# uw-x/AcousticSwarms-Speech

Measured on AMD Instinct MI355X. Metric: TDoA candidates/sec (shift+normalise+spot forward+energies), higher is better.
Workload: dtype f32 via f16x3 split-operand MFMA (fp32 accumulate); 1 GPU; configs[2] scene: 5-speaker reverberant mixture (image sources), 7 mics, T=48000 samples (BASELINE's '3 s @ 16 kHz' sample count; the reference pipeline and this scene generator run at 48 kHz, where it is a 1 s clip -- the reference-native 3 s is extras.T144000), fine-stage (Strict=1) candidate batch of one mixture, FULL spot net 47.27 M params, seeded random weights; internal_batch=256, parallelism=candidate-shard x1

## Files before the change

acousticswarms-speech_amd/csrc/asw_common.h:

```cpp
#pragma once
#include <hip/hip_runtime.h>

#include <cstdarg>
#include <cstdio>
#include <cstring>

#include "../../include/asw_hip.h"

namespace asw {

char* err_buf();
int set_error(int code, const char* fmt, ...);

#define ASW_CHECK_ARG(cond, ...)                                   \
  do {                                                             \
    if (!(cond)) return ::asw::set_error(ASW_ERR_ARG, __VA_ARGS__); \
  } while (0)

#define ASW_HIP(call)                                                                 \
  do {                                                                                \
    hipError_t _e = (call);                                                           \
    if (_e != hipSuccess)                                                             \
      return ::asw::set_error(ASW_ERR_HIP, "%s failed: %s (%s:%d)", #call,            \
                              hipGetErrorString(_e), __FILE__, __LINE__);             \
  } while (0)

#define ASW_LAUNCH_CHECK()                                                            \
  do {                                                                                \
    hipError_t _e = hipGetLastError();                                                \
    if (_e != hipSuccess)                                                             \
      return ::asw::set_error(ASW_ERR_HIP, "kernel launch failed: %s (%s:%d)",        \
                              hipGetErrorString(_e), __FILE__, __LINE__);             \
  } while (0)

static inline hipStream_t as_stream(void* s) { return reinterpret_cast<hipStream_t>(s); }

struct SmemAttr {
  static constexpr int kMaxDev = 64;
  size_t bytes[kMaxDev] = {};
  int ensure(const void* kern, size_t want);
};
static inline int cdiv(long a, long b) { return (int)((a + b - 1) / b); }

#ifdef __HIPCC__
__device__ __forceinline__ float gn_glu_value(float a, float g, float m0, float r0, float m1, float r1, float ga, float ba,
                                              float gg, float bg) {
  const float av = __fmaf_rn(__fmul_rn(__fsub_rn(a, m0), r0), ga, ba);
  const float gv = __fmaf_rn(__fmul_rn(__fsub_rn(g, m1), r1), gg, bg);
  const float e = __builtin_amdgcn_exp2f(__fmul_rn(gv, -1.4426950408889634f));
  return __fmul_rn(av, __builtin_amdgcn_rcpf(__fadd_rn(1.0f, e)));
}
#endif

}

#include <string>
namespace asw {
std::string prof_name(const char* base, int bm, int bn, int bk, bool ln, bool stats);
bool prof_detail();
struct ProfScope {
  ProfScope(hipStream_t s, const std::string& name, double work, double bytes = 0.0);
  ~ProfScope();
  int slot;
  hipStream_t stream;
};
}
```

acousticswarms-speech_amd/csrc/model_common.h:

```cpp
#pragma once
#include <cstdlib>
#include <iterator>
#include <map>
#include <memory>
#include <string>
#include <vector>

#include "asw_common.h"

namespace asw_model {

struct DevBuf {
  float* p = nullptr;
  size_t n = 0;
  DevBuf() = default;
  DevBuf(const DevBuf&) = delete;
  DevBuf& operator=(const DevBuf&) = delete;
  DevBuf(DevBuf&& o) noexcept : p(o.p), n(o.n) { o.p = nullptr; o.n = 0; }
  ~DevBuf() { if (p) (void)hipFree(p); }
  int upload(const std::vector<float>& h) {
    if (p) { (void)hipFree(p); p = nullptr; }
    n = h.size();
    if (hipMalloc(&p, n * sizeof(float)) != hipSuccess) return asw::set_error(ASW_ERR_NOMEM, "hipMalloc(%zu floats)", n);
    ASW_HIP(hipMemcpy(p, h.data(), n * sizeof(float), hipMemcpyHostToDevice));
    return ASW_OK;
  }
};

struct WBuf {
  DevBuf f32;
  uint16_t* hi = nullptr;
  uint16_t* lo = nullptr;
  int32_t shift = 0;
  WBuf() = default;
  WBuf(const WBuf&) = delete;
  WBuf& operator=(const WBuf&) = delete;
  WBuf(WBuf&& o) noexcept : f32(std::move(o.f32)), hi(o.hi), lo(o.lo), shift(o.shift), fhi(o.fhi), flo(o.flo) {
    o.hi = o.lo = o.fhi = o.flo = nullptr;
  }
  ~WBuf() {
    if (hi) (void)hipFree(hi);
    if (lo) (void)hipFree(lo);
    if (fhi) (void)hipFree(fhi);
    if (flo) (void)hipFree(flo);
  }
  int upload_gemm(const std::vector<float>& h, int N, int K) {
    int rc = upload(h);
    if (rc) return rc;
    if (N % 32 == 0 && K % 16 == 0 && (size_t)N * K == h.size()) return upload_frags(h, N, K);
    return ASW_OK;
  }
  int upload(const std::vector<float>& h) {
    int rc = f32.upload(h);
    if (rc) return rc;
    std::vector<uint16_t> vh(h.size()), vl(h.size());
    if ((rc = asw_split_weights_f16(h.data(), h.size(), vh.data(), vl.data(), &shift))) return rc;
    if (hi) { (void)hipFree(hi); hi = nullptr; }
    if (lo) { (void)hipFree(lo); lo = nullptr; }
    if (hipMalloc(&hi, h.size() * 2) != hipSuccess || hipMalloc(&lo, h.size() * 2) != hipSuccess)
      return asw::set_error(ASW_ERR_NOMEM, "hipMalloc(%zu halves)", h.size());
    ASW_HIP(hipMemcpy(hi, vh.data(), h.size() * 2, hipMemcpyHostToDevice));
    ASW_HIP(hipMemcpy(lo, vl.data(), h.size() * 2, hipMemcpyHostToDevice));
    return ASW_OK;
  }
  uint16_t* fhi = nullptr;
  uint16_t* flo = nullptr;
  int upload_frags(const std::vector<float>& h, int N, int K) {
    std::vector<uint16_t> vh(h.size()), vl(h.size());
    int32_t sh = 0;
    int rc = asw_pack_fragments_f16(h.data(), N, K, vh.data(), vl.data(), &sh);
    if (rc) return rc;
    if (sh != shift) return asw::set_error(ASW_ERR_STATE, "fragment pack: inconsistent weight shift");
    if (fhi) { (void)hipFree(fhi); fhi = nullptr; }
    if (flo) { (void)hipFree(flo); flo = nullptr; }
    if (hipMalloc(&fhi, h.size() * 2) != hipSuccess || hipMalloc(&flo, h.size() * 2) != hipSuccess)
      return asw::set_error(ASW_ERR_NOMEM, "hipMalloc(%zu halves)", h.size());
    ASW_HIP(hipMemcpy(fhi, vh.data(), h.size() * 2, hipMemcpyHostToDevice));
    ASW_HIP(hipMemcpy(flo, vl.data(), h.size() * 2, hipMemcpyHostToDevice));
    return ASW_OK;
  }
  void bind(asw_convgemm_args& a, int precision) const {
    a.Wt = f32.p; a.Wt_hi = hi; a.Wt_lo = lo; a.w_shift = shift; a.precision = precision;
    a.Wf_hi = fhi; a.Wf_lo = flo;
  }
};

struct ResLayer { WBuf wt; DevBuf bias, g, b; int dil = 1; };

inline std::vector<float> pack_conv(const std::vector<float>& w, int N, int Cin, int K, const float* in_gate) {
  std::vector<float> o((size_t)N * Cin * K);
  for (int n = 0; n < N; ++n)
    for (int c = 0; c < Cin; ++c)
      for (int k = 0; k < K; ++k)
        o[((size_t)n * K + k) * Cin + c] = w[((size_t)n * Cin + c) * K + k] * (in_gate ? in_gate[c] : 1.f);
  return o;
}


inline int pack_res_layers(const std::map<std::string, std::vector<float>>& raw, const std::string& p, int ch, int K,
                           int n_layers, int dil_factor, std::vector<ResLayer>& out) {
  out.clear();
  out.resize(n_layers);
  int dil = 1;
  for (int j = 0; j < n_layers; ++j) {
    const std::string q = p + ".res.seq." + std::to_string(j);
    int rc;
    {
      const std::vector<float> packed = pack_conv(raw.at(q + ".conv.weight"), ch, ch, K, nullptr);
      if ((rc = out[j].wt.upload(packed))) return rc;
      if (ch % 32 == 0 && (ch * K) % 16 == 0 && (rc = out[j].wt.upload_frags(packed, ch, ch * K))) return rc;
    }
    if ((rc = out[j].bias.upload(raw.at(q + ".conv.bias")))) return rc;
    if ((rc = out[j].g.upload(raw.at(q + ".norm.weight")))) return rc;
    if ((rc = out[j].b.upload(raw.at(q + ".norm.bias")))) return rc;
    out[j].dil = dil;
    dil *= dil_factor;
  }
  return ASW_OK;
}

struct Arena {
  char* base;
  size_t off = 0, cap;
  bool dry;
  Arena(char* b, size_t c, bool d) : base(b), cap(c), dry(d) {}
  template <typename T>
  T* take(size_t n) {
    off = (off + 255) & ~(size_t)255;
    T* p = reinterpret_cast<T*>(base + off);
    off += n * sizeof(T);
    return p;
  }
};


struct GluSrc { const float* raw; const float* mr; const float* gamma; const float* beta; float* side_out = nullptr; };

inline bool glu_on_load_ok(const std::vector<ResLayer>& res, int prec, int ch) {
  static const int max_c = getenv("ASW_GLU_ON_LOAD_MAX_C") ? atoi(getenv("ASW_GLU_ON_LOAD_MAX_C")) : 512;
  return prec >= 1 && (ch == 64 || ch == 128 || ch == 256 || ch == 512) && ch <= max_c && !res.empty() &&
         res[0].dil == 1 && res[0].wt.fhi && res[0].wt.flo;
}

inline bool resstack_ok(const std::vector<ResLayer>& res, int prec, int ch, int K) {
  static const bool off = getenv("ASW_NO_RESSTACK") != nullptr;
  if (off || prec < 1 || ch != 64 || K % 2 == 0 || K < 3 || K > 15) return false;
  for (const ResLayer& r : res)
    if (!r.wt.fhi || !r.wt.flo) return false;
  return true;
}

inline int run_res(const std::vector<ResLayer>& res, int prec, int B, int T, int ch, int K, float* x, float* p, float* q,
            float** final_out, hipStream_t s, const GluSrc* glu = nullptr) {
  const float* in = glu ? glu->raw : x;
  float* outb = p;
  if (resstack_ok(res, prec, ch, K)) {
    static const bool nofuse = getenv("ASW_RESSTACK_NOFUSE") != nullptr;
    size_t j = 0;
    while (j < res.size()) {
      size_t n = 1;
      int halo = 0;
      while (!nofuse && j + n < res.size() && n < 3) {
        const int pad = res[j + n].dil * (K - 1) / 2;
        if (halo + pad > 64) break;
        halo += pad;
        ++n;
      }
      asw_resstack_args a = {};
      a.x = (glu && j == 0) ? nullptr : in;
      a.out = outb;
      a.B = B; a.T = T; a.C = ch; a.taps = K; a.n_layers = (int)n; a.precision = prec; a.ln_eps = 1e-5f;
      for (size_t i = 0; i < n; ++i) {
        const ResLayer& r = res[j + i];
        a.layer[i].Wf_hi = r.wt.fhi; a.layer[i].Wf_lo = r.wt.flo; a.layer[i].w_shift = r.wt.shift;
        a.layer[i].bias = r.bias.p; a.layer[i].ln_gamma = r.g.p; a.layer[i].ln_beta = r.b.p; a.layer[i].dil = r.dil;
      }
      if (glu && j == 0) {
        a.glu_raw = glu->raw; a.glu_mr = glu->mr; a.glu_gamma = glu->gamma; a.glu_beta = glu->beta; a.glu_out = glu->side_out;
      }
      int rc = asw_resstack64_f16x3(&a, s);
      if (rc) return rc;
      in = outb;
      outb = (outb == p) ? q : p;
      j += n;
    }
    *final_out = const_cast<float*>(in);
    return ASW_OK;
  }
  for (size_t j = 0; j < res.size(); ++j) {
    asw_convgemm_args a = {};
    a.A = in; res[j].wt.bind(a, prec); a.bias = res[j].bias.p; a.resid = in;
    if (glu && j == 0) {
      a.glu_raw = glu->raw; a.glu_mr = glu->mr; a.glu_gamma = glu->gamma; a.glu_beta = glu->beta; a.glu_out = glu->side_out;
    }
    a.ln_gamma = res[j].g.p; a.ln_beta = res[j].b.p; a.out = outb;
    a.B = B; a.M_out = T; a.N = ch; a.Cin = ch; a.taps = K; a.stride = 1; a.dil = res[j].dil;
    a.pad = (res[j].dil * (K - 1) + 1) / 2;
    a.a_row_stride = ch; a.a_batch_stride = (int64_t)T * ch; a.a_len = (int64_t)T * ch;
    a.relu = 1; a.ln_eps = 1e-5f;
    int rc = asw_convgemm_f32(&a, s);
    if (rc) return rc;
    in = outb;
    outb = (outb == p) ? q : p;
  }
  *final_out = const_cast<float*>(in);
  return ASW_OK;
}

inline int linear(const float* A, const WBuf& W, int prec, const float* bias, int rows, int N, int K, int relu, const float* resid,
           const float* g, const float* b, float* out, hipStream_t s) {
  asw_convgemm_args a = {};
  a.A = A; W.bind(a, prec); a.bias = bias; a.resid = resid; a.ln_gamma = g; a.ln_beta = b; a.out = out;
  a.B = 1; a.M_out = rows; a.N = N; a.Cin = K; a.taps = 1; a.stride = 1; a.dil = 1; a.pad = 0;
  a.a_row_stride = K; a.a_batch_stride = (int64_t)rows * K; a.a_len = (int64_t)rows * K;
  a.relu = relu; a.ln_eps = 1e-5f;
  if (g && N >= 1024 && N % 256 == 0 && N <= 2048) {
    a.resid = nullptr; a.ln_gamma = nullptr; a.ln_beta = nullptr;
    int rc = asw_convgemm_f32(&a, s);
    if (rc) return rc;
    return asw_add_layernorm(out, resid, g, b, rows, N, 1e-5f, out, s);
  }
  return asw_convgemm_f32(&a, s);
}

inline void pack_conv_transpose(const std::vector<float>& w, const std::vector<float>& b, int Cin, int N, int S,
                                const float* out_gate, std::vector<float>& wt, std::vector<float>& bb) {
  wt.assign((size_t)S * N * Cin, 0.f);
  bb.assign((size_t)S * N, 0.f);
  for (int r = 0; r < S; ++r)
    for (int n = 0; n < N; ++n) {
      bb[(size_t)r * N + n] = out_gate ? b[n] * out_gate[n] : b[n];
      for (int c = 0; c < Cin; ++c) {
        const float v = w[((size_t)c * N + n) * S + r];
        wt[((size_t)r * N + n) * Cin + c] = out_gate ? v * out_gate[n] : v;
      }
    }
}


#define UP(buf, vec) if ((rc = (buf).upload(vec))) return rc

struct TrunkCfg {
  int n_mics, kernel_size, depth, stride_list[8], channels, growth, encoder_channels, encoder_kernel_size,
      encoder_stride, residual_layers, residual_dilation_factor, ffw_dim;
  template <class Cfg>
  static TrunkCfg of(const Cfg& c) {
    TrunkCfg t = {c.n_mics, c.kernel_size, c.depth, {}, c.channels, c.growth, c.encoder_channels,
                  c.encoder_kernel_size, c.encoder_stride, c.residual_layers, c.residual_dilation_factor, c.ffw_dim};
    for (int i = 0; i < 8; ++i) t.stride_list[i] = c.stride_list[i];
    return t;
  }
};

inline int check_trunk_config(const TrunkCfg& c, const char* who, const char* odd) {
  ASW_CHECK_ARG(c.depth >= 1 && c.depth <= 8, "%s: depth %d", who, c.depth);
  ASW_CHECK_ARG(c.n_mics >= 1 && c.n_mics <= 32, "%s: n_mics %d", who, c.n_mics);
  ASW_CHECK_ARG(c.channels % 64 == 0, "%s: channels=%d must be a multiple of 64 for the MFMA tiles", who, c.channels);
  ASW_CHECK_ARG(c.growth >= 1 && c.residual_layers >= 1, "%s: bad config", who);
  ASW_CHECK_ARG(c.kernel_size % 2 == 1, "%s: %s", who, odd);
  ASW_CHECK_ARG(c.encoder_channels % 128 == 0, "%s: encoder_channels must be a multiple of 128", who);
  ASW_CHECK_ARG(c.encoder_stride % 4 == 0 && c.encoder_kernel_size / 2 == c.encoder_stride && c.encoder_kernel_size <= 64,
                "%s: encoder kernel/stride %d/%d unsupported (the reference's trim [9:-8] assumes 33/16)", who,
                c.encoder_kernel_size, c.encoder_stride);
  ASW_CHECK_ARG(c.ffw_dim % 128 == 0, "%s: ffw_dim must be a multiple of 128", who);
  return ASW_OK;
}

struct EncBlock { std::vector<ResLayer> res; DevBuf bias, gn_g, gn_b; };
struct DecBlock { std::vector<ResLayer> res; DevBuf gn_g, gn_b; };
struct GatedConvs { std::vector<WBuf> down_wt, up_wt; std::vector<DevBuf> up_bias; };
struct Tap { const float* p; size_t numel; };
using ParamList = std::vector<std::pair<std::string, size_t>>;

struct TrunkPlan {
  int B, T, Tp, F, RL;
  std::vector<int> Tl;
  float *mean, *stdv, *refn;
  std::vector<float*> X, Pb, Qb, raw_dn, raw_up, st_dn, st_up, mr_dn, mr_up;
  float *Y, *D, *ywave;
};

struct Trunk {
  TrunkCfg tc;
  std::map<std::string, std::vector<float>> raw;
  std::map<std::string, Tap> taps;
  bool finalized = false;
  int device = 0;
  int precision = 0;
  bool fuse_mask = true;

  std::vector<int> enc_cin, enc_cout;
  std::vector<int> dec_cin, dec_cout, dec_stride;
  int stride_product = 1;

  DevBuf pre_w, pre_b;
  std::vector<EncBlock> enc;
  std::vector<DecBlock> dec;
  WBuf byp_wt, mask_wt, dec_wt;
  WBuf byp_wt48;
  DevBuf byp_b, mask_b;
  float out_bias = 0.f;
  int byp_k = 0;

  const std::vector<float>& P(const std::string& k) const { return raw.at(k); }

  int init_shape(const TrunkCfg& c, const char* who) {
    tc = c;
    ASW_HIP(hipGetDevice(&device));
    int cin = c.channels, ch = c.channels;
    for (int i = 0; i < c.depth; ++i) {
      ASW_CHECK_ARG(c.stride_list[i] >= 1, "%s: stride", who);
      enc_cin.push_back(cin);
      enc_cout.push_back(ch);
      stride_product *= c.stride_list[i];
      cin = ch;
      ch *= c.growth;
    }
    dec_cin.assign(enc_cout.rbegin(), enc_cout.rend());
    dec_cout.assign(enc_cin.rbegin(), enc_cin.rend());
    dec_stride.assign(std::make_reverse_iterator(c.stride_list + c.depth), std::make_reverse_iterator(c.stride_list));
    return ASW_OK;
  }
  int check_level_widths(const char* who) const {
    for (int w : enc_cin) ASW_CHECK_ARG(w <= 512 && (w & (w - 1)) == 0, "%s: level width %d must be a power of two <= 512", who, w);
    return ASW_OK;
  }

  ParamList trunk_params() const {
    ParamList v;
    const size_t K = tc.kernel_size;
    v.push_back({"preproc.weight", (size_t)tc.channels * tc.n_mics});
    v.push_back({"preproc.bias", (size_t)tc.channels});
    auto res = [&](const std::string& p, size_t ch) {
      for (int j = 0; j < tc.residual_layers; ++j) {
        const std::string q = p + ".res.seq." + std::to_string(j);
        v.push_back({q + ".conv.weight", ch * ch * K});
        v.push_back({q + ".conv.bias", ch});
        v.push_back({q + ".norm.weight", ch});
        v.push_back({q + ".norm.bias", ch});
      }
    };
    for (int i = 0; i < tc.depth; ++i) {
      const std::string p = "encoder.module_list." + std::to_string(i);
      const size_t ci = enc_cin[i], co = enc_cout[i];
      res(p, ci);
      v.push_back({p + ".conv1.weight", 2 * co * ci * K});
      v.push_back({p + ".conv1.bias", 2 * co});
      v.push_back({p + ".norm1.weight", 2 * co});
      v.push_back({p + ".norm1.bias", 2 * co});
    }
    for (int i = 0; i < tc.depth; ++i) {
      const std::string p = "decoder.module_list." + std::to_string(i);
      const size_t ci = dec_cin[i], co = dec_cout[i], s = dec_stride[i];
      v.push_back({p + ".upsample.conv.weight", ci * 2 * co * s});
      v.push_back({p + ".upsample.conv.bias", 2 * co});
      v.push_back({p + ".norm1.weight", 2 * co});
      v.push_back({p + ".norm1.bias", 2 * co});
      res(p, co);
    }
    const size_t E = tc.encoder_channels, EK = tc.encoder_kernel_size;
    v.push_back({"reference_bypass.weight", E * EK});
    v.push_back({"reference_bypass.bias", E});
    v.push_back({"mask_encoder.weight", E * tc.channels * EK});
    v.push_back({"mask_encoder.bias", E});
    v.push_back({"output_decoder.weight", E * EK});
    v.push_back({"output_decoder.bias", 1});
    return v;
  }

  int finalize_trunk(const char* who, const ParamList& want) {
    {
      int dev = -1;
      ASW_HIP(hipGetDevice(&dev));
      if (dev != device)
        return asw::set_error(ASW_ERR_STATE, "%s: model was created on HIP device %d, current device is %d", who, device, dev);
    }
    for (const auto& kv : want) {
      auto it = raw.find(kv.first);
      if (it == raw.end()) return asw::set_error(ASW_ERR_STATE, "state dict is missing key %s", kv.first.c_str());
      if (it->second.size() != kv.second)
        return asw::set_error(ASW_ERR_ARG, "%s: %zu elements, expected %zu", kv.first.c_str(), it->second.size(), kv.second);
    }
    if (raw.size() != want.size())
      return asw::set_error(ASW_ERR_ARG, "state dict has %zu unexpected keys", raw.size() - want.size());
    int rc;
    const int K = tc.kernel_size, RL = tc.residual_layers, RD = tc.residual_dilation_factor;
    UP(pre_w, P("preproc.weight"));
    UP(pre_b, P("preproc.bias"));
    enc.clear(); enc.resize(tc.depth);
    dec.clear(); dec.resize(tc.depth);
    for (int i = 0; i < tc.depth; ++i) {
      const std::string p = "encoder.module_list." + std::to_string(i);
      if ((rc = pack_res_layers(raw, p, enc_cin[i], K, RL, RD, enc[i].res))) return rc;
      UP(enc[i].bias, P(p + ".conv1.bias"));
      UP(enc[i].gn_g, P(p + ".norm1.weight"));
      UP(enc[i].gn_b, P(p + ".norm1.bias"));
    }
    for (int i = 0; i < tc.depth; ++i) {
      const std::string p = "decoder.module_list." + std::to_string(i);
      if ((rc = pack_res_layers(raw, p, dec_cout[i], K, RL, RD, dec[i].res))) return rc;
      UP(dec[i].gn_g, P(p + ".norm1.weight"));
      UP(dec[i].gn_b, P(p + ".norm1.bias"));
    }
    const int E = tc.encoder_channels, EK = tc.encoder_kernel_size;
    byp_k = ((EK + 31) / 32) * 32;
    {
      const std::vector<float>& w = P("reference_bypass.weight");
      std::vector<float> wt((size_t)E * byp_k, 0.f);
      for (int n = 0; n < E; ++n)
        for (int k = 0; k < EK; ++k) wt[(size_t)n * byp_k + k] = w[(size_t)n * EK + k];
      UP(byp_wt, wt);
      UP(byp_b, P("reference_bypass.bias"));
      if (E % 32 == 0 && EK <= 48) {
        std::vector<float> w48((size_t)E * 48, 0.f);
        for (int n = 0; n < E; ++n)
          for (int k = 0; k < EK; ++k) w48[(size_t)n * 48 + k] = w[(size_t)n * EK + k];
        if ((rc = byp_wt48.upload_gemm(w48, E, 48))) return rc;
      }
    }
    if ((rc = mask_wt.upload_gemm(pack_conv(P("mask_encoder.weight"), E, tc.channels, EK, nullptr), E, tc.channels * EK))) return rc;
    UP(mask_b, P("mask_encoder.bias"));
    {
      const std::vector<float>& w = P("output_decoder.weight");
      std::vector<float> wt((size_t)64 * E, 0.f);
      for (int j = 0; j < EK; ++j)
        for (int e = 0; e < E; ++e) wt[(size_t)j * E + e] = w[(size_t)e * EK + j];
      if ((rc = dec_wt.upload_gemm(wt, 64, E))) return rc;
      out_bias = P("output_decoder.bias")[0];
    }
    return ASW_OK;
  }

  template <class Gate>
  int pack_gated(GatedConvs& o, Gate gate) const {
    const int K = tc.kernel_size;
    int rc;
    o.down_wt.clear(); o.down_wt.resize(tc.depth);
    o.up_wt.clear(); o.up_wt.resize(tc.depth);
    o.up_bias.clear(); o.up_bias.resize(tc.depth);
    for (int i = 0; i < tc.depth; ++i) {
      const std::string p = "encoder.module_list." + std::to_string(i);
      const std::vector<float> g = gate(p);
      const int n = 2 * enc_cout[i], ci = enc_cin[i];
      if ((rc = o.down_wt[i].upload_gemm(pack_conv(P(p + ".conv1.weight"), n, ci, K, g.empty() ? nullptr : g.data()), n, ci * K)))
        return rc;
    }
    for (int j = 0; j < tc.depth; ++j) {
      const std::string p = "decoder.module_list." + std::to_string(j);
      const std::vector<float> g = gate(p);
      const int ci = dec_cin[j], co2 = 2 * dec_cout[j], s = dec_stride[j];
      std::vector<float> wt, bb;
      pack_conv_transpose(P(p + ".upsample.conv.weight"), P(p + ".upsample.conv.bias"), ci, co2, s,
                          g.empty() ? nullptr : g.data(), wt, bb);
      if ((rc = o.up_wt[j].upload_gemm(wt, s * co2, ci))) return rc;
      UP(o.up_bias[j], bb);
    }
    return ASW_OK;
  }

  bool fused_mask_path() const {
    return fuse_mask && precision >= 1 && tc.encoder_channels % 256 == 0 && tc.channels % 32 == 0 &&
           tc.encoder_kernel_size <= 48 && tc.encoder_stride % 4 == 0 && byp_wt48.fhi && dec_wt.fhi && mask_wt.fhi;
  }
  void layout_levels(int B, int T, Arena& a, TrunkPlan& pl) const {
    const int depth = tc.depth, EK = tc.encoder_kernel_size, ES = tc.encoder_stride;
    pl.B = B; pl.T = T;
    pl.Tp = ((T - 1) / stride_product + 1) * stride_product;
    pl.F = (pl.Tp + 2 * (EK / 2) - EK) / ES + 1;
    pl.RL = ((EK / 2 + pl.Tp + byp_k + 64) + 3) & ~3;
    pl.Tl.assign(depth + 1, pl.Tp);
    for (int i = 0; i < depth; ++i) pl.Tl[i + 1] = pl.Tl[i] / tc.stride_list[i];
    pl.mean = a.take<float>(B);
    pl.stdv = a.take<float>(B);
    pl.refn = a.take<float>((size_t)B * pl.RL);
    pl.X.resize(depth + 1); pl.Pb.resize(depth); pl.Qb.resize(depth);
    pl.raw_dn.resize(depth); pl.raw_up.resize(depth); pl.st_dn.resize(depth); pl.st_up.resize(depth);
    pl.mr_up.resize(depth); pl.mr_dn.resize(depth);
    for (int i = 0; i <= depth; ++i) {
      const int ch = i == 0 ? tc.channels : enc_cout[i - 1];
      pl.X[i] = a.take<float>((size_t)B * pl.Tl[i] * ch);
    }
    for (int i = 0; i < depth; ++i) {
      const size_t n = (size_t)B * pl.Tl[i] * enc_cin[i];
      pl.Pb[i] = a.take<float>(n);
      pl.Qb[i] = a.take<float>(n);
      pl.raw_dn[i] = a.take<float>((size_t)B * pl.Tl[i + 1] * 2 * enc_cout[i]);
      pl.st_dn[i] = a.take<float>((size_t)B * 4 * asw_convgemm_stats_tiles(pl.Tl[i + 1], 2 * enc_cout[i]));
      pl.mr_dn[i] = a.take<float>((size_t)B * 4);
    }
    for (int j = 0; j < depth; ++j) {
      const int lvl = depth - j;
      const int s = dec_stride[j], co2 = 2 * dec_cout[j];
      pl.raw_up[j] = a.take<float>((size_t)B * pl.Tl[lvl] * s * co2);
      pl.st_up[j] = a.take<float>((size_t)B * 4 * asw_convgemm_stats_tiles(pl.Tl[lvl], s * co2));
      pl.mr_up[j] = a.take<float>((size_t)B * 4);
    }
  }
  void layout_mask(Arena& a, TrunkPlan& pl) const {
    const int E = tc.encoder_channels;
    const bool fused = fused_mask_path();
    pl.Y = fused ? nullptr : a.take<float>((size_t)pl.B * pl.F * E);
    pl.D = a.take<float>((size_t)(fused ? E / 256 : 1) * pl.B * pl.F * 64);
    pl.ywave = a.take<float>((size_t)pl.B * pl.T);
  }

  int encode(TrunkPlan& pl, const GatedConvs& g, hipStream_t s) {
    const int B = pl.B, K = tc.kernel_size;
    taps.clear();
    taps["preproc"] = {pl.X[0], (size_t)B * pl.Tl[0] * tc.channels};
    int rc;
    GluSrc src = {};
    bool glu = false;
    for (int i = 0; i < tc.depth; ++i) {
      float* r = nullptr;
      if ((rc = run_res(enc[i].res, precision, B, pl.Tl[i], enc_cin[i], K, pl.X[i], pl.Pb[i], pl.Qb[i], &r, s,
                        glu ? &src : nullptr)))
        return rc;
      asw_convgemm_args a = {};
      a.A = r; g.down_wt[i].bind(a, precision); a.bias = enc[i].bias.p; a.out = pl.raw_dn[i]; a.stats = pl.st_dn[i];
      a.B = B; a.M_out = pl.Tl[i + 1]; a.N = 2 * enc_cout[i]; a.Cin = enc_cin[i]; a.taps = K;
      a.stride = tc.stride_list[i]; a.dil = 1; a.pad = K / 2;
      a.a_row_stride = a.Cin; a.a_batch_stride = (int64_t)pl.Tl[i] * a.Cin; a.a_len = a.a_batch_stride;
      a.chan_mod = a.N;
      if ((rc = asw_convgemm_f32(&a, s))) return rc;
      glu = fuse_mask && i + 1 < tc.depth && glu_on_load_ok(enc[i + 1].res, precision, enc_cout[i]);
      const int tiles = asw_convgemm_stats_tiles(a.M_out, a.N);
      if (glu) {
        if ((rc = asw_gn_finalize(pl.st_dn[i], tiles, B, pl.Tl[i + 1], enc_cout[i], 1e-5f, pl.mr_dn[i], s))) return rc;
        src = {pl.raw_dn[i], pl.mr_dn[i], enc[i].gn_g.p, enc[i].gn_b.p, pl.X[i + 1]};
      } else if ((rc = asw_gn_glu(pl.raw_dn[i], pl.st_dn[i], tiles, enc[i].gn_g.p, enc[i].gn_b.p, B, pl.Tl[i + 1],
                                  enc_cout[i], 1e-5f, pl.X[i + 1], s))) {
        return rc;
      }
      taps["enc" + std::to_string(i)] = {pl.X[i + 1], (size_t)B * pl.Tl[i + 1] * enc_cout[i]};
    }
    return ASW_OK;
  }

  int decode(TrunkPlan& pl, const GatedConvs& g, const float*& x, hipStream_t s) {
    const int B = pl.B, K = tc.kernel_size;
    int rc;
    for (int j = 0; j < tc.depth; ++j) {
      const int lvl = tc.depth - j, ci = dec_cin[j], co = dec_cout[j], st = dec_stride[j];
      asw_convgemm_args a = {};
      a.A = x; a.A2 = pl.X[lvl]; g.up_wt[j].bind(a, precision); a.bias = g.up_bias[j].p; a.out = pl.raw_up[j];
      a.stats = pl.st_up[j];
      a.B = B; a.M_out = pl.Tl[lvl]; a.N = st * 2 * co; a.Cin = ci; a.taps = 1; a.stride = 1; a.dil = 1; a.pad = 0;
      a.a_row_stride = ci; a.a_batch_stride = (int64_t)pl.Tl[lvl] * ci; a.a_len = a.a_batch_stride;
      a.chan_mod = 2 * co;
      if ((rc = asw_convgemm_f32(&a, s))) return rc;
      const int To = pl.Tl[lvl] * st;
      const int tiles = asw_convgemm_stats_tiles(a.M_out, a.N);
      float* gb = pl.Qb[lvl - 1];
      float* r = nullptr;
      if (fuse_mask && glu_on_load_ok(dec[j].res, precision, co)) {
        if ((rc = asw_gn_finalize(pl.st_up[j], tiles, B, To, co, 1e-5f, pl.mr_up[j], s))) return rc;
        const GluSrc src = {pl.raw_up[j], pl.mr_up[j], dec[j].gn_g.p, dec[j].gn_b.p, co > 64 ? gb : nullptr};
        if ((rc = run_res(dec[j].res, precision, B, To, co, K, gb, pl.Pb[lvl - 1], gb, &r, s, &src))) return rc;
      } else {
        if ((rc = asw_gn_glu(pl.raw_up[j], pl.st_up[j], tiles, dec[j].gn_g.p, dec[j].gn_b.p, B, To, co, 1e-5f, gb, s)))
          return rc;
        if ((rc = run_res(dec[j].res, precision, B, To, co, K, gb, pl.Pb[lvl - 1], gb, &r, s))) return rc;
      }
      x = r;
      taps["dec" + std::to_string(j)] = {x, (size_t)B * To * co};
    }
    return ASW_OK;
  }

  int mask_path(TrunkPlan& pl, const float* x, const float* mean, const float* stdv, float* out_wave, hipStream_t s) {
    const int B = pl.B, C = tc.channels, E = tc.encoder_channels, EK = tc.encoder_kernel_size, ES = tc.encoder_stride;
    int rc;
    asw_convgemm_args me = {};
    me.A = x; mask_wt.bind(me, precision); me.bias = mask_b.p;
    me.B = B; me.M_out = pl.F; me.N = E; me.Cin = C; me.taps = EK; me.stride = ES; me.dil = 1; me.pad = EK / 2;
    me.a_row_stride = C; me.a_batch_stride = (int64_t)pl.Tp * C; me.a_len = me.a_batch_stride;
    if (fused_mask_path()) {
      asw_maskpath_args f = {};
      f.enc = me;
      f.ref = pl.refn; f.ref_batch_stride = pl.RL; f.ref_len = pl.RL; f.ref_hop = ES;
      f.byp_k = 48; f.byp_taps = EK; f.byp_shift = byp_wt48.shift; f.byp_hi = byp_wt48.fhi; f.byp_lo = byp_wt48.flo;
      f.byp_bias = byp_b.p;
      f.dec_hi = dec_wt.fhi; f.dec_lo = dec_wt.flo; f.dec_shift = dec_wt.shift; f.dec_taps = EK;
      f.taps = pl.D;
      if ((rc = asw_mask_path_f16x3(&f, s))) return rc;
      return asw_overlap_add_parts(pl.D, E / 256, B, pl.F, 64, EK, EK / 2, pl.T, 9, 8, out_bias, mean, stdv, out_wave, s);
    }
    {
      asw_convgemm_args a = {};
      a.A = pl.refn; byp_wt.bind(a, precision); a.bias = byp_b.p; a.out = pl.Y;
      a.B = B; a.M_out = pl.F; a.N = E; a.Cin = byp_k; a.taps = 1; a.stride = 1; a.dil = 1; a.pad = 0;
      a.a_row_stride = ES; a.a_batch_stride = pl.RL; a.a_len = pl.RL; a.relu = 1;
      if ((rc = asw_convgemm_f32(&a, s))) return rc;
    }
    me.mul = pl.Y; me.out = pl.Y; me.relu = 1;
    if ((rc = asw_convgemm_f32(&me, s))) return rc;
    taps["latent"] = {pl.Y, (size_t)B * pl.F * E};
    {
      asw_convgemm_args a = {};
      a.A = pl.Y; dec_wt.bind(a, precision); a.out = pl.D;
      a.B = B; a.M_out = pl.F; a.N = 64; a.Cin = E; a.taps = 1; a.stride = 1; a.dil = 1; a.pad = 0;
      a.a_row_stride = E; a.a_batch_stride = (int64_t)pl.F * E; a.a_len = a.a_batch_stride;
      if ((rc = asw_convgemm_f32(&a, s))) return rc;
    }
    return asw_overlap_add_unnorm(pl.D, B, pl.F, 64, EK, EK / 2, pl.T, 9, 8, out_bias, mean, stdv, out_wave, s);
  }
};

inline int check_ready(const Trunk* m, const char* fin) {
  if (!m) return asw::set_error(ASW_ERR_ARG, "null model handle");
  if (!m->finalized) return asw::set_error(ASW_ERR_STATE, "%s() has not been called", fin);
  int dev = -1;
  ASW_HIP(hipGetDevice(&dev));
  if (dev != m->device)
    return asw::set_error(ASW_ERR_STATE, "model lives on HIP device %d but the current device is %d", m->device, dev);
  return ASW_OK;
}

inline int set_precision(Trunk* m, const char* who, int precision) {
  ASW_CHECK_ARG(m && (precision >= 0 && precision <= 2), "%s: 0 (f32), 1 (f16x3) or 2 (single-pass f16)", who);
  m->precision = precision;
  return ASW_OK;
}

inline int set_param(Trunk* m, const char* who, const char* key, const float* host_data, size_t numel) {
  ASW_CHECK_ARG(m && key && host_data, "%s: null pointer", who);
  m->raw[key].assign(host_data, host_data + numel);
  m->finalized = false;
  return ASW_OK;
}

inline int get_tap(const Trunk* m, const char* who, const char* name, float* dst, size_t capacity, size_t* numel,
                   void* stream) {
  ASW_CHECK_ARG(m && name && numel, "%s: null pointer", who);
  auto it = m->taps.find(name);
  if (it == m->taps.end()) return asw::set_error(ASW_ERR_ARG, "%s: no activation named %s", who, name);
  *numel = it->second.numel;
  if (dst) {
    ASW_CHECK_ARG(capacity >= it->second.numel, "%s: buffer too small", who);
    ASW_HIP(hipMemcpyAsync(dst, it->second.p, it->second.numel * sizeof(float), hipMemcpyDeviceToDevice,
                           asw::as_stream(stream)));
  }
  return ASW_OK;
}

}
```

acousticswarms-speech_amd/csrc/prep_kernels.hip:

```cpp
#include "asw_common.h"

namespace {

constexpr int MAX_MICS = 32;

__device__ __forceinline__ float quant16(float x) {
  return rintf(x * 32768.0f) * (1.0f / 32768.0f);
}

__device__ __forceinline__ double block_sum(double v, double* red) {
#pragma unroll
  for (int o = 32; o > 0; o >>= 1) v += __shfl_xor(v, o, 64);
  const int lane = threadIdx.x & 63, wid = threadIdx.x >> 6, nw = blockDim.x >> 6;
  __syncthreads();
  if (lane == 0) red[wid] = v;
  __syncthreads();
  double s = 0.0;
  for (int i = 0; i < nw; ++i) s += red[i];
  return s;
}

__global__ __launch_bounds__(1024) void shift_stats_kernel(const float* __restrict__ mixes, int M, int T,
                                                           const int32_t* __restrict__ offsets,
                                                           const int32_t* __restrict__ mix_index, int circular,
                                                           float* __restrict__ mean_out,
                                                           float* __restrict__ std_out) {
  __shared__ int off[MAX_MICS];
  __shared__ double red[16];
  const int n = blockIdx.x;
  const float* __restrict__ mix = mixes + (mix_index ? (long)mix_index[n] * M * T : 0);
  if (threadIdx.x < M) {
    int o = threadIdx.x == 0 ? 0 : offsets[(long)n * (M - 1) + threadIdx.x - 1];
    if (circular) { o %= T; if (o < 0) o += T; }
    off[threadIdx.x] = o;
  }
  __syncthreads();
  const float inv_m = 1.0f / (float)M;
  auto ref_at = [&](int t) -> float {
    float s = 0.f;
    for (int m = 0; m < M; ++m) {
      int i = t + off[m];
      float x;
      if (circular) { if (i >= T) i -= T; x = mix[(long)m * T + i]; }
      else x = (i >= 0 && i < T) ? mix[(long)m * T + i] : 0.f;
      s += quant16(x);
    }
    return s * inv_m;
  };
  double acc = 0.0;
  for (int t = threadIdx.x; t < T; t += blockDim.x) acc += (double)ref_at(t);
  const double mean = block_sum(acc, red) / (double)T;
  acc = 0.0;
  for (int t = threadIdx.x; t < T; t += blockDim.x) {
    const double d = (double)ref_at(t) - mean;
    acc += d * d;
  }
  const double var = block_sum(acc, red) / (double)(T - 1);
  if (threadIdx.x == 0) {
    mean_out[n] = (float)mean;
    std_out[n] = (float)sqrt(var);
  }
}

template <bool SHIFTED>
__global__ __launch_bounds__(256) void preproc_kernel(const float* __restrict__ srcs, int M, int T, int T_pad,
                                                      const int32_t* __restrict__ offsets,
                                                      const int32_t* __restrict__ mix_index, int circular,
                                                      const float* __restrict__ mean, const float* __restrict__ stdv,
                                                      const float* __restrict__ w, const float* __restrict__ bias,
                                                      int C, float* __restrict__ x0, float* __restrict__ refn,
                                                      long refn_stride, int rows_per_block) {
  __shared__ int off[MAX_MICS];
  __shared__ float vs[64 * MAX_MICS];
  __shared__ float ws[128 * MAX_MICS];
  const int n = blockIdx.y;
  const float* __restrict__ src = srcs + ((SHIFTED && mix_index) ? (long)mix_index[n] * M * T : 0);
  for (int i = threadIdx.x; i < C * M; i += blockDim.x) ws[i] = w[i];
  const int c4n = C >> 2;
  if (threadIdx.x < M) {
    int o = 0;
    if (SHIFTED && threadIdx.x > 0) {
      o = offsets[(long)n * (M - 1) + threadIdx.x - 1];
      if (circular) { o %= T; if (o < 0) o += T; }
    }
    off[threadIdx.x] = o;
  }
  __syncthreads();
  const int pad = T_pad - T;
  const float mu = SHIFTED ? mean[n] : 0.f;
  const float sg = SHIFTED ? stdv[n] : 1.f;
  const int row0 = blockIdx.x * rows_per_block;
  for (int it = threadIdx.x; it < rows_per_block * M; it += blockDim.x) {
    const int m = it / rows_per_block, r = it - m * rows_per_block;
    const int tp = row0 + r;
    float x = 0.f;
    if (tp >= pad && tp < T_pad) {
      const int t = tp - pad;
      if (SHIFTED) {
        int i = t + off[m];
        if (circular) { if (i >= T) i -= T; x = src[(long)m * T + i]; }
        else x = (i >= 0 && i < T) ? src[(long)m * T + i] : 0.f;
        x = (quant16(x) - mu) / sg;
      } else {
        x = src[((long)n * M + m) * T + t];
      }
    }
    vs[r * M + m] = x;
  }
  __syncthreads();
  const int items = rows_per_block * c4n;
  for (int it = threadIdx.x; it < items; it += blockDim.x) {
    const int r = it / c4n, c4 = it - r * c4n;
    const int tp = row0 + r;
    if (tp >= T_pad) break;
    const int c = c4 * 4;
    float4 o = *reinterpret_cast<const float4*>(bias + c);
    if (tp >= pad) {
      for (int m = 0; m < M; ++m) {
        const float x = vs[r * M + m];
        o.x = fmaf(ws[(c + 0) * M + m], x, o.x);
        o.y = fmaf(ws[(c + 1) * M + m], x, o.y);
        o.z = fmaf(ws[(c + 2) * M + m], x, o.z);
        o.w = fmaf(ws[(c + 3) * M + m], x, o.w);
      }
    }
    *reinterpret_cast<float4*>(x0 + ((long)n * T_pad + tp) * C + c) = o;
    if (c4 == 0) refn[(long)n * refn_stride + tp] = vs[r * M];
  }
}

}

extern "C" int asw_shift_stats(const float* mix, int M, int T, const int32_t* offsets, int N, int circular,
                               float* mean, float* std, void* stream) {
  return asw_shift_stats_multi(mix, M, T, offsets, nullptr, N, circular, mean, std, stream);
}

extern "C" int asw_shift_stats_multi(const float* mix, int M, int T, const int32_t* offsets, const int32_t* mix_index, int N,
                                     int circular, float* mean, float* std, void* stream) {
  ASW_CHECK_ARG(mix && offsets && mean && std, "shift_stats: null pointer");
  ASW_CHECK_ARG(M >= 1 && M <= MAX_MICS && T >= 2, "shift_stats: M=%d T=%d unsupported", M, T);
  if (N == 0) return ASW_OK;
  asw::ProfScope prof(asw::as_stream(stream), "shift_stats", 0.0, (double)M * T * 4 + (double)N * 8);
  hipLaunchKernelGGL(shift_stats_kernel, dim3(N), dim3(1024), 0, asw::as_stream(stream), mix, M, T, offsets, mix_index,
                     circular, mean, std);
  ASW_LAUNCH_CHECK();
  return ASW_OK;
}

extern "C" int asw_shift_norm_preproc(const float* mix, int M, int T, int T_pad, const int32_t* offsets, int N,
                                      int circular, const float* mean, const float* std, const float* w,
                                      const float* b, int C, float* x0, float* refn, long refn_stride,
                                      void* stream) {
  return asw_shift_norm_preproc_multi(mix, M, T, T_pad, offsets, nullptr, N, circular, mean, std, w, b, C, x0, refn,
                                      refn_stride, stream);
}

extern "C" int asw_shift_norm_preproc_multi(const float* mix, int M, int T, int T_pad, const int32_t* offsets,
                                            const int32_t* mix_index, int N, int circular, const float* mean,
                                            const float* std, const float* w, const float* b, int C, float* x0, float* refn,
                                            long refn_stride, void* stream) {
  ASW_CHECK_ARG(refn_stride >= T_pad, "shift_norm_preproc: refn_stride < T_pad");
  ASW_CHECK_ARG(mix && offsets && mean && std && w && b && x0 && refn, "shift_norm_preproc: null pointer");
  ASW_CHECK_ARG(M >= 1 && M <= MAX_MICS && T >= 1 && T_pad >= T && C % 4 == 0 && C > 0 && C <= 128,
                "shift_norm_preproc: bad shape M=%d T=%d T_pad=%d C=%d (C <= 128)", M, T, T_pad, C);
  if (N == 0) return ASW_OK;
  const int rows = 64;
  dim3 grid(asw::cdiv(T_pad, rows), N);
  asw::ProfScope prof(asw::as_stream(stream), "preproc", 0.0, (double)M * T * 4 + (double)N * T_pad * (C + 1) * 4);
  hipLaunchKernelGGL(preproc_kernel<true>, grid, dim3(256), 0, asw::as_stream(stream), mix, M, T, T_pad, offsets, mix_index,
                     circular, mean, std, w, b, C, x0, refn, refn_stride, rows);
  ASW_LAUNCH_CHECK();
  return ASW_OK;
}

extern "C" int asw_pad_preproc(const float* x, int B, int M, int t, int T_pad, const float* w, const float* b,
                               int C, float* x0, float* refn, long refn_stride, void* stream) {
  ASW_CHECK_ARG(refn_stride >= T_pad, "pad_preproc: refn_stride < T_pad");
  ASW_CHECK_ARG(x && w && b && x0 && refn, "pad_preproc: null pointer");
  ASW_CHECK_ARG(M >= 1 && M <= MAX_MICS && t >= 1 && T_pad >= t && C % 4 == 0 && C > 0 && C <= 128,
                "pad_preproc: bad shape M=%d t=%d T_pad=%d C=%d (C <= 128)", M, t, T_pad, C);
  if (B == 0) return ASW_OK;
  const int rows = 64;
  dim3 grid(asw::cdiv(T_pad, rows), B);
  hipLaunchKernelGGL(preproc_kernel<false>, grid, dim3(256), 0, asw::as_stream(stream), x, M, t, T_pad,
                     (const int32_t*)nullptr, (const int32_t*)nullptr, 1, (const float*)nullptr, (const float*)nullptr, w, b, C, x0, refn,
                     refn_stride, rows);
  ASW_LAUNCH_CHECK();
  return ASW_OK;
}
```

acousticswarms-speech_amd/csrc/resstack.hip:

```cpp
#include <cstdlib>
#include <type_traits>

#include "asw_common.h"
#include "mfma_util.h"

namespace {
using namespace asw_mfma;

constexpr int RS = 272;
constexpr int C = 64;
constexpr int MAXL = 3;

struct LayerDev {
  const half8* Wh;
  const half8* Wl;
  const float* bias;
  const float* gamma;
  const float* beta;
  int dil, pad;
  int halo;
  int nfrag;
  float scale;
};

#ifdef ASW_PHASE_TIMING
__device__ unsigned long long g_rs_cycles[6] = {0, 0, 0, 0, 0, 0};
#define RS_MARK(var) const unsigned long long var = __builtin_readcyclecounter()
#else
#define RS_MARK(var)
#endif

struct KArgs {
  const float* x;
  float* out;
  const float* glu_raw;
  const float* glu_mr;
  const float* glu_gamma;
  const float* glu_beta;
  float* glu_out;
  int B, T, taps, ntile, BM, img_rows;
  float eps;
  LayerDev L[MAXL];
};

template <int NF, int QD, int NTERM>
__device__ __forceinline__ void kloop(floatx16 (&acc)[NF][2], const char* img, const int (&xb)[NF], int taps, int tapstep,
                                      const half8* __restrict__ Wh, const half8* __restrict__ Wl, int lane) {
  auto wload = [&](int kg, half8 (&h)[2], half8 (&l)[2]) {
#pragma unroll
    for (int cb = 0; cb < 2; ++cb) {
      const long o = ((long)kg * 2 + cb) * 64 + lane;
      h[cb] = Wh[o];
      if (NTERM == 3) l[cb] = Wl[o];
    }
  };
  auto xload = [&](int tap, int ks, half8 (&h)[NF], half8 (&l)[NF]) {
#pragma unroll
    for (int i = 0; i < NF; ++i) {
      const char* q = img + xb[i] + tap * tapstep + ks * 32;
      h[i] = *reinterpret_cast<const half8*>(q);
      if (NTERM == 3) l[i] = *reinterpret_cast<const half8*>(q + 128);
    }
  };
  half8 wh[QD][2], wl[QD][2];
  half8 xh[2][NF], xl[2][NF];
#pragma unroll
  for (int q = 0; q < QD; ++q) wload(q, wh[q], wl[q]);
  xload(0, 0, xh[0], xl[0]);
  const int nks = taps * 4;
  for (int tap = 0; tap < taps; ++tap) {
#pragma unroll
    for (int ks = 0; ks < 4; ++ks) {
      const int nk = (ks + 1) & 3;
      int nt = tap + (ks == 3 ? 1 : 0);
      nt = nt < taps ? nt : taps - 1;
      xload(nt, nk, xh[(ks + 1) & 1], xl[(ks + 1) & 1]);
      __builtin_amdgcn_sched_barrier(0);
      const int s = ks % QD, xbuf = ks & 1;
#pragma unroll
      for (int i = 0; i < NF; ++i)
#pragma unroll
        for (int cb = 0; cb < 2; ++cb) {
          if (NTERM == 3) {
            acc[i][cb] = __builtin_amdgcn_mfma_f32_32x32x16_f16(wh[s][cb], xl[xbuf][i], acc[i][cb], 0, 0, 0);
            acc[i][cb] = __builtin_amdgcn_mfma_f32_32x32x16_f16(wl[s][cb], xh[xbuf][i], acc[i][cb], 0, 0, 0);
          }
          acc[i][cb] = __builtin_amdgcn_mfma_f32_32x32x16_f16(wh[s][cb], xh[xbuf][i], acc[i][cb], 0, 0, 0);
        }
      int kg = tap * 4 + ks + QD;
      kg = kg < nks ? kg : nks - 1;
      wload(kg, wh[s], wl[s]);
      __builtin_amdgcn_sched_barrier(0);
    }
  }
}

template <int NL, int NW, int TM, int PH, bool POLY, bool GLU, int NTERM, int QD>
__global__ __launch_bounds__(64 * NW) __attribute__((amdgpu_waves_per_eu(TM >= 4 ? 1 : 2)))
void resstack64_kernel(const KArgs p) {
  static_assert(!POLY || NL == 1, "polyphase row sets: single layers only");
  static_assert(QD == 2 || QD == 4, "weight prefetch depth in k-steps");
  constexpr int NTHR = 64 * NW, SROWS = NTHR / 16;
  constexpr int R0 = 32 * NW * TM;
  constexpr int BMJ = R0 / PH;
  static_assert(BMJ % 32 == 0, "a row fragment must stay inside one phase");

  extern __shared__ __align__(16) char smem[];
  char* img = smem;
  float* tab = reinterpret_cast<float*>(smem + (size_t)p.img_rows * RS);

  const int tid = threadIdx.x, lane = tid & 63, wid = tid >> 6;
  const int total = p.B * p.ntile;
  const int per = (total + 7) >> 3;
  const int idx = (int)(blockIdx.x & 7) * per + (int)(blockIdx.x >> 3);
  if (idx >= total) return;
  const int b = idx / p.ntile, tile = idx - b * p.ntile;
  const int T = p.T, taps = p.taps;
  const int dil0 = p.L[0].dil, pad0 = p.L[0].pad;
  const int n_pb = POLY ? (dil0 + PH - 1) / PH : 1;
  const int jb = POLY ? tile / n_pb : 0, pb = POLY ? tile - jb * n_pb : 0;
  const int m0 = tile * p.BM;
  const int RJ = BMJ + taps - 1;
  const int R_img = POLY ? PH * RJ : R0 + 2 * pad0;

  RS_MARK(t_start);
  for (int i = tid; i < NL * 3 * 16; i += NTHR) {
    const int li = i / 48, w = (i - li * 48) / 16, c4 = i & 15;
    const float* src = w == 0 ? p.L[li].bias : w == 1 ? p.L[li].gamma : p.L[li].beta;
    reinterpret_cast<float4*>(tab)[i] = *reinterpret_cast<const float4*>(src + c4 * 4);
  }
  {
    const __amdgpu_buffer_rsrc_t rX = GLU ? act_rsrc(p.glu_raw + (long)b * T * 2 * C, (long)T * 2 * C)
                                          : act_rsrc(p.x + (long)b * T * C, (long)T * C);
    const int srow = tid >> 4, sc4 = tid & 15;
    float gm0 = 0.f, gr0 = 0.f, gm1 = 0.f, gr1 = 0.f;
    float4 gga, gba, ggg, gbg;
    if (GLU) {
      gm0 = p.glu_mr[b * 4 + 0]; gr0 = p.glu_mr[b * 4 + 1]; gm1 = p.glu_mr[b * 4 + 2]; gr1 = p.glu_mr[b * 4 + 3];
      gga = *reinterpret_cast<const float4*>(p.glu_gamma + sc4 * 4);
      gba = *reinterpret_cast<const float4*>(p.glu_beta + sc4 * 4);
      ggg = *reinterpret_cast<const float4*>(p.glu_gamma + C + sc4 * 4);
      gbg = *reinterpret_cast<const float4*>(p.glu_beta + C + sc4 * 4);
    }
    constexpr int SU = GLU ? 9 : 18;
    for (int r0 = 0; r0 < R_img; r0 += SROWS * SU) {
      float4 buf[SU];
      float4 gate[GLU ? SU : 1];
      bool okr[GLU ? SU : 1];
#pragma unroll
      for (int u = 0; u < SU; ++u) {
        const int row = r0 + u * SROWS + srow;
        int g;
        bool ok = row < R_img;
        if (!POLY) {
          g = m0 - p.L[0].halo - pad0 + row;
        } else {
          const int ph = pb * PH + row / RJ;
          const int jj = jb * BMJ + row % RJ - (taps - 1) / 2;
          g = dil0 * jj + ph;
          ok = ok && ph < dil0 && jj >= 0;
        }
        ok = ok && g >= 0 && g < T;
        if (GLU) {
          buf[u] = act_load4(rX, (long)g * 2 * C + sc4 * 4, ok);
          gate[u] = act_load4(rX, (long)g * 2 * C + C + sc4 * 4, ok);
          okr[u] = ok;
        } else {
          buf[u] = act_load4(rX, (long)g * C + sc4 * 4, ok);
        }
      }
      if (GLU) {
#pragma unroll
        for (int u = 0; u < SU; ++u) {
          float4 o;
#define ASW_GLU(f)                                                       \
  {                                                                      \
    const float gl = asw::gn_glu_value(buf[u].f, gate[u].f, gm0, gr0, gm1, gr1, gga.f, gba.f, ggg.f, gbg.f); \
    o.f = okr[u] ? gl : 0.f;                                             \
  }
          ASW_GLU(x) ASW_GLU(y) ASW_GLU(z) ASW_GLU(w)
#undef ASW_GLU
          buf[u] = o;
          if (p.glu_out && okr[u]) {
            const int g = m0 - p.L[0].halo - pad0 + r0 + u * SROWS + srow;
            if (g >= m0 && g < m0 + p.BM)
              *reinterpret_cast<float4*>(p.glu_out + ((long)b * T + g) * C + sc4 * 4) = o;
          }
        }
      }
#pragma unroll
      for (int u = 0; u < SU; ++u) {
        const int row = r0 + u * SROWS + srow;
        if (row < R_img) {
          half4 hi, lo;
          split4t<NTERM>(buf[u], hi, lo);
          *reinterpret_cast<half4*>(img + row * RS + sc4 * 8) = hi;
          *reinterpret_cast<half4*>(img + row * RS + 128 + sc4 * 8) = lo;
        }
      }
    }
  }
  __syncthreads();
  RS_MARK(t_staged);
#ifdef ASW_PHASE_TIMING
  unsigned long long t_marks[2 * MAXL + 1];
  t_marks[0] = t_staged;
#endif

  const int h = lane >> 5;
  floatx16 acc[TM][2];
  auto layer = [&](auto lic) {
    constexpr int li = decltype(lic)::value;
    constexpr bool last = li == NL - 1;
    const LayerDev& Ld = p.L[li];
    const int tapstep = (POLY ? 1 : Ld.dil) * RS;
    const int nf = Ld.nfrag - wid * TM;
#pragma unroll
    for (int i = 0; i < TM; ++i)
#pragma unroll
      for (int cb = 0; cb < 2; ++cb)
#pragma unroll
        for (int r = 0; r < 16; ++r) acc[i][cb][r] = 0.f;
    auto img_row = [&](int trow) { return POLY ? (trow / BMJ) * RJ + trow % BMJ : trow; };
    auto run = [&](auto nfc) {
      constexpr int NF = decltype(nfc)::value;
      int xb[NF];
      floatx16 a[NF][2];
#pragma unroll
      for (int i = 0; i < NF; ++i) {
        xb[i] = (img_row((wid * TM + i) * 32) + (lane & 31)) * RS + h * 16;
        a[i][0] = acc[i][0];
        a[i][1] = acc[i][1];
      }
      kloop<NF, QD, NTERM>(a, img, xb, taps, tapstep, Ld.Wh, Ld.Wl, lane);
#pragma unroll
      for (int i = 0; i < NF; ++i) { acc[i][0] = a[i][0]; acc[i][1] = a[i][1]; }
    };
    if (nf >= TM) run(std::integral_constant<int, TM>{});
    else if constexpr (TM > 1) {
      if (nf == 1) run(std::integral_constant<int, 1>{});
      if constexpr (TM > 2) {
        if (nf == 2) run(std::integral_constant<int, 2>{});
        if (nf == 3) run(std::integral_constant<int, 3>{});
      }
    }
#ifdef ASW_PHASE_TIMING
    {
      float sink = acc[0][0][0];
      asm volatile("" ::"v"(sink));
      t_marks[2 * li + 1] = __builtin_readcyclecounter();
    }
#endif
    const float* tb = tab + li * 192;
    const int cpad = POLY ? (taps - 1) / 2 : Ld.pad;
#pragma unroll
    for (int i = 0; i < TM; ++i) {
      if (i < nf) {
        const int trow = (wid * TM + i) * 32 + (lane & 31);
        const char* rrow = img + (img_row(trow) + cpad) * RS;
        float s = 0.f;
#pragma unroll
        for (int cb = 0; cb < 2; ++cb)
#pragma unroll
          for (int q = 0; q < 4; ++q) {
            const int c0 = cb * 32 + q * 8 + h * 4;
            const float4 bi = *reinterpret_cast<const float4*>(tb + c0);
            const half4 rh = *reinterpret_cast<const half4*>(rrow + c0 * 2);
            const half4 rl = *reinterpret_cast<const half4*>(rrow + 128 + c0 * 2);
            const float bv[4] = {bi.x, bi.y, bi.z, bi.w};
#pragma unroll
            for (int j = 0; j < 4; ++j) {
              float v = fmaxf(acc[i][cb][q * 4 + j] * Ld.scale + bv[j], 0.f);
              v += (float)rh[j] + (float)rl[j];
              acc[i][cb][q * 4 + j] = v;
              s += v;
            }
          }
        s += __shfl_xor(s, 32, 64);
        const float mean = s * (1.0f / C);
        float d = 0.f;
#pragma unroll
        for (int cb = 0; cb < 2; ++cb)
#pragma unroll
          for (int r = 0; r < 16; ++r) { const float cx = acc[i][cb][r] - mean; d += cx * cx; }
        d += __shfl_xor(d, 32, 64);
        const float rstd = 1.0f / sqrtf(d * (1.0f / C) + p.eps);
#pragma unroll
        for (int cb = 0; cb < 2; ++cb)
#pragma unroll
          for (int q = 0; q < 4; ++q) {
            const int c0 = cb * 32 + q * 8 + h * 4;
            const float4 g4 = *reinterpret_cast<const float4*>(tb + 64 + c0);
            const float4 b4 = *reinterpret_cast<const float4*>(tb + 128 + c0);
            const float gv[4] = {g4.x, g4.y, g4.z, g4.w}, be[4] = {b4.x, b4.y, b4.z, b4.w};
#pragma unroll
            for (int j = 0; j < 4; ++j) acc[i][cb][q * 4 + j] = (acc[i][cb][q * 4 + j] - mean) * rstd * gv[j] + be[j];
          }
      }
    }
    if constexpr (!last) {
      __syncthreads();
#pragma unroll
      for (int i = 0; i < TM; ++i) {
        if (i < nf) {
          const int trow = (wid * TM + i) * 32 + (lane & 31);
          const int t = m0 - Ld.halo + trow;
          const bool inside = t >= 0 && t < T;
          char* wrow = img + trow * RS;
#pragma unroll
          for (int cb = 0; cb < 2; ++cb)
#pragma unroll
            for (int q = 0; q < 4; ++q) {
              const int c0 = cb * 32 + q * 8 + h * 4;
              float4 v = make_float4(acc[i][cb][q * 4 + 0], acc[i][cb][q * 4 + 1], acc[i][cb][q * 4 + 2], acc[i][cb][q * 4 + 3]);
              if (!inside) v = make_float4(0.f, 0.f, 0.f, 0.f);
              half4 hi, lo;
              split4t<NTERM>(v, hi, lo);
              *reinterpret_cast<half4*>(wrow + c0 * 2) = hi;
              *reinterpret_cast<half4*>(wrow + 128 + c0 * 2) = lo;
            }
        }
      }
      __syncthreads();
    } else {
      float* __restrict__ ob = p.out + (long)b * T * C;
#pragma unroll
      for (int i = 0; i < TM; ++i) {
        if (i < nf) {
          const int trow = (wid * TM + i) * 32 + (lane & 31);
          int t;
          bool ok;
          if (!POLY) {
            t = m0 + trow;
            ok = trow < p.BM && t < T;
          } else {
            const int ph = pb * PH + trow / BMJ;
            t = dil0 * (jb * BMJ + trow % BMJ) + ph;
            ok = ph < dil0 && t < T;
          }
          if (ok) {
            float* orow = ob + (long)t * C;
#pragma unroll
            for (int cb = 0; cb < 2; ++cb)
#pragma unroll
              for (int q = 0; q < 4; ++q) {
                const int c0 = cb * 32 + q * 8 + h * 4;
                *reinterpret_cast<float4*>(orow + c0) =
                    make_float4(acc[i][cb][q * 4 + 0], acc[i][cb][q * 4 + 1], acc[i][cb][q * 4 + 2], acc[i][cb][q * 4 + 3]);
              }
          }
        }
      }
    }
  };
  layer(std::integral_constant<int, 0>{});
#ifdef ASW_PHASE_TIMING
  t_marks[2] = __builtin_readcyclecounter();
#endif
  if constexpr (NL > 1) layer(std::integral_constant<int, 1>{});
  if constexpr (NL > 2) layer(std::integral_constant<int, 2>{});
#ifdef ASW_PHASE_TIMING
  if (threadIdx.x == 0 && NL <= 2) {
    const unsigned long long t_end = __builtin_readcyclecounter();
    atomicAdd(&g_rs_cycles[0], t_staged - t_start);
    atomicAdd(&g_rs_cycles[1], t_marks[1] - t_marks[0]);
    if (NL == 1) {
      atomicAdd(&g_rs_cycles[4], t_end - t_marks[1]);
    } else {
      atomicAdd(&g_rs_cycles[2], t_marks[2] - t_marks[1]);
      atomicAdd(&g_rs_cycles[3], t_marks[3] - t_marks[2]);
      atomicAdd(&g_rs_cycles[4], t_end - t_marks[3]);
    }
    atomicAdd(&g_rs_cycles[5], 1ull);
  }
#endif
}

template <int NL, int NW, int TM, int PH, bool POLY, bool GLU, int QD>
int launch_stack(const KArgs& k, int precision, size_t smem, double flops, const char* tag, hipStream_t s) {
  const bool x1 = precision == 2;
  auto kern = x1 ? resstack64_kernel<NL, NW, TM, PH, POLY, GLU, 1, QD> : resstack64_kernel<NL, NW, TM, PH, POLY, GLU, 3, QD>;
  static asw::SmemAttr attr[2];
  if (int rc = attr[x1].ensure(reinterpret_cast<const void*>(kern), 160 * 1024)) return rc;
  const int total = k.B * k.ntile;
  dim3 grid(((total + 7) / 8) * 8);
  char nm[128];
  int nl = snprintf(nm, sizeof nm, "resstack64<%s,%dx%d%s%s>", tag, NW, TM, POLY ? (PH == 1 ? ",poly1" : PH == 2 ? ",poly2" : ",poly4") : "",
                    GLU ? ",glu" : "");
  if (asw::prof_detail()) snprintf(nm + nl, sizeof nm - nl, "[B%d M%d d%d]", k.B, k.T, k.L[0].dil);
  asw::ProfScope prof(s, nm, flops, (double)k.B * k.T * C * 4 * (GLU ? 3 : 2));
  hipLaunchKernelGGL(kern, grid, dim3(64 * NW), smem, s, k);
  ASW_LAUNCH_CHECK();
  return ASW_OK;
}

template <int NW, int TM>
int dispatch(const asw_resstack_args& a, KArgs& k, bool glu, double flops, hipStream_t s) {
  constexpr int R0 = 32 * NW * TM;
  const int dil0 = k.L[0].dil;
  const int rpp = a.T / dil0;
  if (a.n_layers == 1 && dil0 >= 7 && rpp >= 48 && !glu) {
    const int PH = rpp >= R0 - 32 ? 1 : rpp >= R0 / 2 - 32 ? 2 : 4;
    const int BMJ = R0 / PH;
    k.BM = R0;
    k.L[0].nfrag = NW * TM;
    k.ntile = asw::cdiv(asw::cdiv(a.T, dil0), BMJ) * asw::cdiv(dil0, PH);
    k.img_rows = PH * (BMJ + a.taps - 1);
    const size_t smem = (size_t)k.img_rows * RS + 3 * 64 * sizeof(float);
    switch (PH) {
      case 1: return launch_stack<1, NW, TM, 1, true, false, 4>(k, a.precision, smem, flops, "1", s);
      case 2: return launch_stack<1, NW, TM, 2, true, false, 4>(k, a.precision, smem, flops, "1", s);
      default: return launch_stack<1, NW, TM, 4, true, false, 4>(k, a.precision, smem, flops, "1", s);
    }
  }
  k.BM = R0 - 2 * k.L[0].halo;
  ASW_CHECK_ARG(k.BM >= R0 / 2, "resstack: the later layers' halo (%d rows per side) leaves %d of %d rows; fuse fewer layers",
                k.L[0].halo, k.BM, R0);
  k.ntile = asw::cdiv(a.T, k.BM);
  int rows = 0;
  for (int i = 0; i < a.n_layers; ++i) {
    k.L[i].nfrag = asw::cdiv(k.BM + 2 * k.L[i].halo, 32);
    const int r = 32 * k.L[i].nfrag + 2 * k.L[i].pad;
    rows = r > rows ? r : rows;
  }
  k.img_rows = rows;
  const size_t smem = (size_t)rows * RS + (size_t)a.n_layers * 3 * 64 * sizeof(float);
  ASW_CHECK_ARG(smem <= 160 * 1024, "resstack: image of %d rows exceeds LDS (dilation %d x %d taps too wide for a contiguous tile)",
                rows, dil0, a.taps);
  switch (a.n_layers) {
    case 1: return glu ? launch_stack<1, NW, TM, 1, false, true, 4>(k, a.precision, smem, flops, "1", s)
                       : launch_stack<1, NW, TM, 1, false, false, 4>(k, a.precision, smem, flops, "1", s);
    case 2: return glu ? launch_stack<2, NW, TM, 1, false, true, 4>(k, a.precision, smem, flops, "2", s)
                       : launch_stack<2, NW, TM, 1, false, false, 4>(k, a.precision, smem, flops, "2", s);
    default: return glu ? launch_stack<3, NW, TM, 1, false, true, 4>(k, a.precision, smem, flops, "3", s)
                        : launch_stack<3, NW, TM, 1, false, false, 4>(k, a.precision, smem, flops, "3", s);
  }
}

}

#ifdef ASW_PHASE_TIMING
extern "C" int asw_debug_resstack_cycles(unsigned long long* out6, int reset) {
  ASW_HIP(hipMemcpyFromSymbol(out6, HIP_SYMBOL(g_rs_cycles), 6 * sizeof(unsigned long long)));
  if (reset) {
    const unsigned long long z[6] = {0, 0, 0, 0, 0, 0};
    ASW_HIP(hipMemcpyToSymbol(HIP_SYMBOL(g_rs_cycles), z, sizeof z));
  }
  return ASW_OK;
}
#endif

extern "C" int asw_resstack64_f16x3(const asw_resstack_args* args, void* stream) {
  ASW_CHECK_ARG(args != nullptr, "resstack: null args");
  const asw_resstack_args& a = *args;
  hipStream_t s = asw::as_stream(stream);
  ASW_CHECK_ARG(a.C == C, "resstack: C=%d (64 only)", a.C);
  ASW_CHECK_ARG(a.n_layers >= 1 && a.n_layers <= MAXL, "resstack: 1..%d layers", MAXL);
  ASW_CHECK_ARG(a.taps >= 3 && a.taps <= 15 && a.taps % 2 == 1, "resstack: taps=%d (odd, 3..15)", a.taps);
  ASW_CHECK_ARG(a.precision == 1 || a.precision == 2, "resstack: precision 1 (f16x3) or 2 (single-pass f16)");
  ASW_CHECK_ARG(a.B > 0 && a.B <= (1 << 20) && a.T > 0 && (int64_t)a.T * 2 * C < ((int64_t)1 << 29), "resstack: bad B / T");
  ASW_CHECK_ARG(a.out && (a.x || a.glu_raw), "resstack: null tensor");
  const bool glu = a.glu_raw != nullptr;
  if (glu) ASW_CHECK_ARG(a.glu_mr && a.glu_gamma && a.glu_beta, "resstack: GroupNorm + GLU on load needs the statistics / affine arrays");
  KArgs k = {};
  k.x = a.x; k.out = a.out; k.glu_raw = a.glu_raw; k.glu_mr = a.glu_mr; k.glu_gamma = a.glu_gamma; k.glu_beta = a.glu_beta;
  k.glu_out = glu ? a.glu_out : nullptr;
  k.B = a.B; k.T = a.T; k.taps = a.taps; k.eps = a.ln_eps;
  int halo = 0;
  for (int i = a.n_layers - 1; i >= 0; --i) {
    const asw_reslayer_desc& d = a.layer[i];
    ASW_CHECK_ARG(d.Wf_hi && d.Wf_lo && d.bias && d.ln_gamma && d.ln_beta && d.dil >= 1, "resstack: layer %d incomplete", i);
    LayerDev& L = k.L[i];
    L.Wh = reinterpret_cast<const half8*>(d.Wf_hi); L.Wl = reinterpret_cast<const half8*>(d.Wf_lo);
    L.bias = d.bias; L.gamma = d.ln_gamma; L.beta = d.ln_beta;
    L.dil = d.dil; L.pad = d.dil * (a.taps - 1) / 2; L.halo = halo;
    L.scale = ldexpf(1.0f, -d.w_shift);
    halo += L.pad;
  }
  const double flops = 2.0 * a.B * (double)a.T * C * C * a.taps * a.n_layers;
  static const int tile_env = getenv("ASW_RESSTACK_TILE") ? atoi(getenv("ASW_RESSTACK_TILE")) : 0;
  const int variant = tile_env == 24 || tile_env == 44 || tile_env == 82 ? tile_env : 42;
  switch (variant) {
    case 24: return dispatch<2, 4>(a, k, glu, flops, s);
    case 44: return dispatch<4, 4>(a, k, glu, flops, s);
    case 82: return dispatch<8, 2>(a, k, glu, flops, s);
    default: return dispatch<4, 2>(a, k, glu, flops, s);
  }
}
```

acousticswarms-speech_amd/csrc/spot_model.hip:

```cpp
#include <map>
#include <memory>
#include <string>
#include <vector>

#include "model_common.h"

using namespace asw_model;

namespace {

struct TfLayer { WBuf w_in, w_out, w1, w2; DevBuf b_in, b_out, b1, b2, n1g, n1b, n2g, n2b; };
struct GateSet : GatedConvs { uint64_t stamp = 0; };

}

struct asw_spot : Trunk {
  asw_spot_config cfg;
  int batch = 32;
  uint64_t clock = 0;
  std::vector<TfLayer> tf;
  std::map<std::pair<float, float>, std::unique_ptr<GateSet>> gates;

  char* ws[2] = {nullptr, nullptr};
  size_t ws_bytes[2] = {0, 0};
  int lanes = 1;
  hipStream_t side = nullptr;
  hipEvent_t ev_fork = nullptr, ev_join = nullptr;

  ~asw_spot() {
    for (char* w : ws) if (w) (void)hipFree(w);
    if (side) (void)hipStreamDestroy(side);
    if (ev_fork) (void)hipEventDestroy(ev_fork);
    if (ev_join) (void)hipEventDestroy(ev_join);
  }
};

namespace {

ParamList expected_params(const asw_spot* m) {
  const asw_spot_config& c = m->cfg;
  ParamList v = m->trunk_params();
  for (int i = 0; i < c.depth; ++i) {
    const std::string p = "encoder.module_list." + std::to_string(i);
    v.push_back({p + ".embed1.weight", (size_t)m->enc_cin[i] * 2});
    v.push_back({p + ".embed1.bias", (size_t)m->enc_cin[i]});
  }
  for (int i = 0; i < c.depth; ++i) {
    const std::string p = "decoder.module_list." + std::to_string(i);
    v.push_back({p + ".embed1.weight", (size_t)2 * m->dec_cout[i] * 2});
    v.push_back({p + ".embed1.bias", (size_t)2 * m->dec_cout[i]});
  }
  const size_t d = m->enc_cout.back(), f = c.ffw_dim;
  for (int l = 0; l < c.num_transformer_layers; ++l) {
    const std::string p = "bottleneck.transf.layers." + std::to_string(l);
    v.push_back({p + ".self_attn.in_proj_weight", 3 * d * d});
    v.push_back({p + ".self_attn.in_proj_bias", 3 * d});
    v.push_back({p + ".self_attn.out_proj.weight", d * d});
    v.push_back({p + ".self_attn.out_proj.bias", d});
    v.push_back({p + ".linear1.weight", f * d});
    v.push_back({p + ".linear1.bias", f});
    v.push_back({p + ".linear2.weight", d * f});
    v.push_back({p + ".linear2.bias", d});
    v.push_back({p + ".norm1.weight", d});
    v.push_back({p + ".norm1.bias", d});
    v.push_back({p + ".norm2.weight", d});
    v.push_back({p + ".norm2.bias", d});
  }
  return v;
}

std::vector<float> gate_of(const std::vector<float>& w, const std::vector<float>& b, float w0, float w1) {
  std::vector<float> g(b.size());
  for (size_t c = 0; c < b.size(); ++c) g[c] = w[2 * c] * w0 + w[2 * c + 1] * w1 + b[c];
  return g;
}

int get_gates(asw_spot* m, float w0, float w1, GateSet** out) {
  auto key = std::make_pair(w0, w1);
  auto it = m->gates.find(key);
  if (it != m->gates.end()) { it->second->stamp = ++m->clock; *out = it->second.get(); return ASW_OK; }
  if (m->gates.size() >= 8) {
    auto lru = m->gates.begin();
    for (auto g = m->gates.begin(); g != m->gates.end(); ++g)
      if (g->second->stamp < lru->second->stamp) lru = g;
    m->gates.erase(lru);
  }
  std::unique_ptr<GateSet> gs(new GateSet());
  gs->stamp = ++m->clock;
  int rc = m->pack_gated(*gs, [&](const std::string& p) {
    return gate_of(m->P(p + ".embed1.weight"), m->P(p + ".embed1.bias"), w0, w1);
  });
  if (rc) return rc;
  *out = gs.get();
  m->gates[key] = std::move(gs);
  return ASW_OK;
}

struct Plan : TrunkPlan {
  float *qkv, *ctx, *x1, *ff, *ha, *hb;
  double* escr;
};

void layout(const asw_spot* m, int B, int T, Arena& a, Plan& pl) {
  m->layout_levels(B, T, a, pl);
  const size_t L = pl.Tl[m->cfg.depth], d = m->enc_cout.back(), rows = (size_t)B * L;
  pl.qkv = a.take<float>(rows * 3 * d);
  pl.ctx = a.take<float>(rows * d);
  pl.x1 = a.take<float>(rows * d);
  pl.ff = a.take<float>(rows * m->cfg.ffw_dim);
  pl.ha = a.take<float>(rows * d);
  pl.hb = a.take<float>(rows * d);
  m->layout_mask(a, pl);
  pl.escr = a.take<double>((size_t)B * (T + 1));
}

int ensure_ws(asw_spot* m, int B, int T, Plan& pl, int lane = 0) {
  Arena dry(nullptr, 0, true);
  layout(m, B, T, dry, pl);
  const size_t need = dry.off + 4096;
  if (need > m->ws_bytes[lane]) {
    size_t want = need;
    if (B < m->batch) {
      Plan full;
      Arena dry_full(nullptr, 0, true);
      layout(m, m->batch, T, dry_full, full);
      want = dry_full.off + 4096;
    }
    if (m->ws[lane]) { ASW_HIP(hipDeviceSynchronize()); (void)hipFree(m->ws[lane]); m->ws[lane] = nullptr; m->ws_bytes[lane] = 0; }
    if (hipMalloc(&m->ws[lane], want) != hipSuccess) {
      (void)hipGetLastError();
      want = need;
      if (hipMalloc(&m->ws[lane], want) != hipSuccess)
        return asw::set_error(ASW_ERR_NOMEM, "workspace of %.1f MiB for batch %d, T=%d", need / 1048576.0, B, T);
    }
    m->ws_bytes[lane] = want;
  }
  Arena real(m->ws[lane], m->ws_bytes[lane], false);
  layout(m, B, T, real, pl);
  return ASW_OK;
}

int run_network(asw_spot* m, Plan& pl, GateSet* gs, const float* mean, const float* stdv, float* out_wave,
                hipStream_t s) {
  const asw_spot_config& c = m->cfg;
  int rc;
  if ((rc = m->encode(pl, *gs, s))) return rc;
  const int L = pl.Tl[c.depth], d = m->enc_cout.back(), rows = pl.B * L;
  const float* h = pl.X[c.depth];
  for (int l = 0; l < c.num_transformer_layers; ++l) {
    TfLayer& t = m->tf[l];
    float* hout = (l % 2 == 0) ? pl.ha : pl.hb;
    if ((rc = linear(h, t.w_in, m->precision, t.b_in.p, rows, 3 * d, d, 0, nullptr, nullptr, nullptr, pl.qkv, s))) return rc;
    if ((rc = asw_attention_prec(pl.qkv, pl.B, L, d, c.num_head, m->precision, pl.ctx, s))) return rc;
    if ((rc = linear(pl.ctx, t.w_out, m->precision, t.b_out.p, rows, d, d, 0, h, t.n1g.p, t.n1b.p, pl.x1, s))) return rc;
    if ((rc = linear(pl.x1, t.w1, m->precision, t.b1.p, rows, c.ffw_dim, d, 1, nullptr, nullptr, nullptr, pl.ff, s))) return rc;
    if ((rc = linear(pl.ff, t.w2, m->precision, t.b2.p, rows, d, c.ffw_dim, 0, pl.x1, t.n2g.p, t.n2b.p, hout, s))) return rc;
    h = hout;
  }
  m->taps["bottleneck"] = {h, (size_t)rows * d};
  if ((rc = m->decode(pl, *gs, h, s))) return rc;
  return m->mask_path(pl, h, mean, stdv, out_wave, s);
}

}

extern "C" int asw_spot_create(const asw_spot_config* cfg, asw_spot** out) {
  ASW_CHECK_ARG(cfg && out, "spot_create: null pointer");
  const asw_spot_config& c = *cfg;
  const TrunkCfg tc = TrunkCfg::of(c);
  int rc = check_trunk_config(tc, "spot_create", "kernel_size must be odd");
  if (rc) return rc;
  ASW_CHECK_ARG(c.num_transformer_layers >= 0, "spot_create: bad config");
  std::unique_ptr<asw_spot> m(new asw_spot());
  m->cfg = c;
  if ((rc = m->init_shape(tc, "spot_create"))) return rc;
  const int d = m->enc_cout.back();
  ASW_CHECK_ARG(d <= 1024 && (d & (d - 1)) == 0, "spot_create: bottleneck width %d must be a power of two <= 1024", d);
  ASW_CHECK_ARG(d % c.num_head == 0 && (d / c.num_head) % 16 == 0 && d / c.num_head <= 128,
                "spot_create: head_dim %d unsupported", d / (c.num_head ? c.num_head : 1));
  if ((rc = m->check_level_widths("spot_create"))) return rc;
  *out = m.release();
  return ASW_OK;
}

extern "C" void asw_spot_destroy(asw_spot* m) { delete m; }

extern "C" int asw_spot_set_precision(asw_spot* m, int precision) { return set_precision(m, "set_precision", precision); }

extern "C" int asw_spot_set_batch(asw_spot* m, int batch) {
  ASW_CHECK_ARG(m && batch >= 1 && batch <= 4096, "set_batch: bad argument");
  m->batch = batch;
  return ASW_OK;
}

extern "C" int asw_spot_set_param(asw_spot* m, const char* key, const float* host_data, size_t numel) {
  return set_param(m, "set_param", key, host_data, numel);
}

extern "C" int asw_spot_finalize(asw_spot* m) {
  ASW_CHECK_ARG(m, "finalize: null handle");
  const asw_spot_config& c = m->cfg;
  int rc = m->finalize_trunk("finalize", expected_params(m));
  if (rc) return rc;
  m->tf.clear(); m->tf.resize(c.num_transformer_layers);
  for (int l = 0; l < c.num_transformer_layers; ++l) {
    const std::string p = "bottleneck.transf.layers." + std::to_string(l);
    TfLayer& t = m->tf[l];
    {
      const int dm = m->enc_cout.back(), ff = c.ffw_dim;
      if ((rc = t.w_in.upload_gemm(m->P(p + ".self_attn.in_proj_weight"), 3 * dm, dm))) return rc;
      if ((rc = t.w_out.upload_gemm(m->P(p + ".self_attn.out_proj.weight"), dm, dm))) return rc;
      if ((rc = t.w1.upload_gemm(m->P(p + ".linear1.weight"), ff, dm))) return rc;
      if ((rc = t.w2.upload_gemm(m->P(p + ".linear2.weight"), dm, ff))) return rc;
    }
    UP(t.b_in, m->P(p + ".self_attn.in_proj_bias"));
    UP(t.b_out, m->P(p + ".self_attn.out_proj.bias"));
    UP(t.b1, m->P(p + ".linear1.bias"));
    UP(t.b2, m->P(p + ".linear2.bias"));
    UP(t.n1g, m->P(p + ".norm1.weight")); UP(t.n1b, m->P(p + ".norm1.bias"));
    UP(t.n2g, m->P(p + ".norm2.weight")); UP(t.n2b, m->P(p + ".norm2.bias"));
  }
  m->gates.clear();
  m->finalized = true;
  return ASW_OK;
}

extern "C" int asw_spot_shift_and_sep(asw_spot* m, const float* mix, int M, int T, const int32_t* offsets, int N,
                                      int strict, int circular, float* out_wave, double* out_energy,
                                      int energy_window, void* stream) {
  return asw_spot_shift_and_sep_multi(m, mix, 1, M, T, offsets, nullptr, N, strict, circular, out_wave, out_energy,
                                      energy_window, stream);
}

extern "C" int asw_spot_shift_and_sep_multi(asw_spot* m, const float* mix, int K, int M, int T, const int32_t* offsets,
                                            const int32_t* mix_index, int N, int strict, int circular, float* out_wave,
                                            double* out_energy, int energy_window, void* stream) {
  int rc = check_ready(m, "asw_spot_finalize");
  ASW_CHECK_ARG(K >= 1 && (K == 1 || mix_index != nullptr), "shift_and_sep: K=%d mixtures need a mix_index array", K);
  if (rc) return rc;
  ASW_CHECK_ARG(N >= 0, "shift_and_sep: N=%d", N);
  if (N == 0) return ASW_OK;
  ASW_CHECK_ARG(mix && offsets, "shift_and_sep: null pointer");
  ASW_CHECK_ARG(M == m->cfg.n_mics, "shift_and_sep: mixture has %d channels, model expects %d", M, m->cfg.n_mics);
  ASW_CHECK_ARG(T >= 2, "shift_and_sep: T=%d", T);
  ASW_CHECK_ARG(out_energy == nullptr || energy_window > 0, "shift_and_sep: energy_window");
  hipStream_t s = asw::as_stream(stream);
  GateSet* gs = nullptr;
  if ((rc = get_gates(m, strict == 1 ? 1.f : 0.f, strict == 1 ? 0.f : 1.f, &gs))) return rc;
  const int Bmax = N < m->batch ? N : m->batch;
  const int n_batches = (N + Bmax - 1) / Bmax;
  const int lanes = (m->lanes == 2 && n_batches >= 2) ? 2 : 1;
  Plan pl[2];
  for (int l = 0; l < lanes; ++l)
    if ((rc = ensure_ws(m, Bmax, T, pl[l], l))) return rc;
  hipStream_t st[2] = {s, s};
  if (lanes == 2) {
    if (!m->side) {
      ASW_HIP(hipStreamCreateWithFlags(&m->side, hipStreamNonBlocking));
      ASW_HIP(hipEventCreateWithFlags(&m->ev_fork, hipEventDisableTiming));
      ASW_HIP(hipEventCreateWithFlags(&m->ev_join, hipEventDisableTiming));
    }
    st[1] = m->side;
    ASW_HIP(hipEventRecord(m->ev_fork, s));
    ASW_HIP(hipStreamWaitEvent(m->side, m->ev_fork, 0));
  }
  const int C = m->cfg.channels, pad_l = m->cfg.encoder_kernel_size / 2;
  auto batches = [&]() -> int {
    int k = 0;
    for (int i0 = 0; i0 < N; i0 += Bmax, ++k) {
      const int B = N - i0 < Bmax ? N - i0 : Bmax;
      Plan& p = pl[k % lanes];
      hipStream_t q = st[k % lanes];
      p.B = B;
      const int32_t* off = offsets + (size_t)i0 * (M - 1);
      const int32_t* mi = mix_index ? mix_index + i0 : nullptr;
      ASW_HIP(hipMemsetAsync(p.refn, 0, (size_t)B * p.RL * sizeof(float), q));
      int r;
      if ((r = asw_shift_stats_multi(mix, M, T, off, mi, B, circular, p.mean, p.stdv, q))) return r;
      if ((r = asw_shift_norm_preproc_multi(mix, M, T, p.Tp, off, mi, B, circular, p.mean, p.stdv, m->pre_w.p, m->pre_b.p, C,
                                            p.X[0], p.refn + pad_l, p.RL, q)))
        return r;
      float* y = out_wave ? out_wave + (size_t)i0 * T : p.ywave;
      if ((r = run_network(m, p, gs, p.mean, p.stdv, y, q))) return r;
      if (out_energy && (r = asw_energies(y, B, T, energy_window, p.escr, out_energy + (size_t)i0 * 2, q))) return r;
    }
    return ASW_OK;
  };
  rc = batches();
  if (lanes == 2) {
    if (hipEventRecord(m->ev_join, m->side) != hipSuccess || hipStreamWaitEvent(s, m->ev_join, 0) != hipSuccess) {
      (void)hipStreamSynchronize(m->side);
      if (!rc) rc = asw::set_error(ASW_ERR_HIP, "shift_and_sep: joining the side lane failed");
    }
  }
  return rc;
}

extern "C" int asw_spot_set_lanes(asw_spot* m, int lanes) {
  ASW_CHECK_ARG(m && (lanes == 1 || lanes == 2), "set_lanes: 1 or 2");
  m->lanes = lanes;
  return ASW_OK;
}

extern "C" int asw_spot_forward(asw_spot* m, const float* mix_norm, int B, int M, int t,
                                const float* window_embedding_host, float* out, void* stream) {
  int rc = check_ready(m, "asw_spot_finalize");
  if (rc) return rc;
  ASW_CHECK_ARG(B >= 0, "forward: B=%d", B);
  if (B == 0) return ASW_OK;
  ASW_CHECK_ARG(mix_norm && window_embedding_host && out, "forward: null pointer");
  ASW_CHECK_ARG(M == m->cfg.n_mics && t >= 1, "forward: bad shape");
  hipStream_t s = asw::as_stream(stream);
  GateSet* gs = nullptr;
  if ((rc = get_gates(m, window_embedding_host[0], window_embedding_host[1], &gs))) return rc;
  const int Bmax = B < m->batch ? B : m->batch;
  Plan pl;
  if ((rc = ensure_ws(m, Bmax, t, pl))) return rc;
  const int C = m->cfg.channels, pad_l = m->cfg.encoder_kernel_size / 2;
  for (int i0 = 0; i0 < B; i0 += Bmax) {
    const int b = B - i0 < Bmax ? B - i0 : Bmax;
    pl.B = b;
    ASW_HIP(hipMemsetAsync(pl.refn, 0, (size_t)b * pl.RL * sizeof(float), s));
    if ((rc = asw_pad_preproc(mix_norm + (size_t)i0 * M * t, b, M, t, pl.Tp, m->pre_w.p, m->pre_b.p, C, pl.X[0],
                              pl.refn + pad_l, pl.RL, s)))
      return rc;
    if ((rc = run_network(m, pl, gs, nullptr, nullptr, out + (size_t)i0 * t, s))) return rc;
  }
  return ASW_OK;
}

extern "C" int asw_spot_set_fused_mask(asw_spot* m, int on) {
  ASW_CHECK_ARG(m, "set_fused_mask: null model handle");
  m->fuse_mask = on != 0;
  return ASW_OK;
}

extern "C" int asw_spot_get_tap(asw_spot* m, const char* name, float* dst, size_t capacity, size_t* numel,
                                void* stream) {
  return get_tap(m, "get_tap", name, dst, capacity, numel, stream);
}
```

acousticswarms-speech_amd/native.py:

```python
import ctypes
import os
import subprocess
import sys
from ctypes import (POINTER, Structure, c_char_p, c_double, c_float, c_int, c_int32, c_int64,
                    c_long, c_size_t, c_void_p)

_HERE = os.path.dirname(os.path.abspath(__file__))
LIB_PATH = os.environ.get("ASW_LIB_PATH") or os.path.join(_HERE, "libasw_hip.so")
CSRC = os.path.join(_HERE, "csrc")
SOURCES = ["asw_common.cpp", "convgemm.hip", "resstack.hip", "downconv.hip", "prep_kernels.hip", "misc_kernels.hip", "attention_mfma.hip", "srp_kernels.hip",
           "pruner_kernels.hip", "geometry_kernels.hip",
           "search_host.cpp", "sep_kernels.hip", "spot_model.hip", "sep_model.hip"]
HEADERS = ["asw_common.h", "model_common.h", "mfma_util.h"]
EXTRA_FLAGS = {"geometry_kernels.hip": ["-ffp-contract=off"]}
OPS_PATH = os.path.join(_HERE, "libasw_torch_ops.so")
OPS_SOURCE = "torch_ops.cpp"


def build(force: bool = False, verbose: bool = False) -> str:
    from concurrent.futures import ThreadPoolExecutor
    hdrs = [os.path.join(CSRC, h) for h in HEADERS] + [os.path.join(os.path.dirname(_HERE), "include", "asw_hip.h")]
    hdr_time = max(os.path.getmtime(h) for h in hdrs)
    objdir = os.path.join(_HERE, "build")
    os.makedirs(objdir, exist_ok=True)
    jobs, objs = [], []
    for src in SOURCES:
        sp = os.path.join(CSRC, src)
        op = os.path.join(objdir, os.path.splitext(src)[0] + ".o")
        objs.append(op)
        if force or not os.path.exists(op) or os.path.getmtime(op) < max(os.path.getmtime(sp), hdr_time):
            jobs.append(["hipcc", "-O3", "--offload-arch=gfx950", "-std=c++17", "-fPIC"] + EXTRA_FLAGS.get(src, [])
                        + ["-c", sp, "-o", op])
    if not jobs and os.path.exists(LIB_PATH) and all(os.path.getmtime(LIB_PATH) >= os.path.getmtime(o) for o in objs):
        return LIB_PATH

    def run(cmd):
        if verbose:
            print(" ".join(cmd), file=sys.stderr)
        subprocess.run(cmd, check=True)
    with ThreadPoolExecutor(max_workers=min(6, max(1, len(jobs)))) as ex:
        list(ex.map(run, jobs))
    run(["hipcc", "--offload-arch=gfx950", "-fPIC", "-shared", "-o", LIB_PATH] + objs)
    return LIB_PATH


def build_torch_ops(force: bool = False, verbose: bool = False) -> str:
    import torch
    src = os.path.join(CSRC, OPS_SOURCE)
    hdr = os.path.join(os.path.dirname(_HERE), "include", "asw_hip.h")
    if not force and os.path.exists(OPS_PATH) and os.path.getmtime(OPS_PATH) >= max(
            os.path.getmtime(src), os.path.getmtime(hdr), os.path.getmtime(LIB_PATH)):
        return OPS_PATH
    ti = os.path.dirname(torch.__file__)
    cmd = ["hipcc", "-O2", "-std=c++17", "-fPIC", "-shared", "-D__HIP_PLATFORM_AMD__=1", "-DUSE_ROCM=1",
           f"-D_GLIBCXX_USE_CXX11_ABI={int(torch._C._GLIBCXX_USE_CXX11_ABI)}", "-w",
           f"-I{ti}/include", f"-I{ti}/include/torch/csrc/api/include", "-I/opt/rocm/include", src, "-o", OPS_PATH,
           f"-L{_HERE}", "-lasw_hip", f"-L{ti}/lib", "-ltorch", "-ltorch_cpu", "-lc10", "-lc10_hip", "-ltorch_hip",
           "-Wl,-rpath,$ORIGIN", f"-Wl,-rpath,{ti}/lib"]
    if verbose:
        print(" ".join(cmd), file=sys.stderr)
    subprocess.run(cmd, check=True)
    return OPS_PATH


class SpotConfigC(Structure):
    _fields_ = [("n_mics", c_int32), ("kernel_size", c_int32), ("depth", c_int32),
                ("stride_list", c_int32 * 8), ("channels", c_int32), ("growth", c_int32),
                ("encoder_channels", c_int32), ("encoder_kernel_size", c_int32),
                ("encoder_stride", c_int32), ("residual_layers", c_int32),
                ("residual_dilation_factor", c_int32), ("num_head", c_int32), ("ffw_dim", c_int32),
                ("num_transformer_layers", c_int32)]

    @classmethod
    def from_config(cls, cfg):
        s = cls()
        s.n_mics, s.kernel_size, s.depth = cfg.n_mics, cfg.kernel_size, cfg.depth
        for i, v in enumerate(cfg.stride_list):
            s.stride_list[i] = v
        s.channels, s.growth = cfg.channels, int(cfg.growth)
        s.encoder_channels, s.encoder_kernel_size = cfg.encoder_channels, cfg.encoder_kernel_size
        s.encoder_stride, s.residual_layers = cfg.encoder_stride, cfg.residual_layers
        s.residual_dilation_factor, s.num_head = cfg.residual_dilation_factor, cfg.num_head
        s.ffw_dim, s.num_transformer_layers = cfg.ffw_dim, cfg.num_transformer_layers
        return s


class SepConfigC(Structure):
    _fields_ = [("n_mics", c_int32), ("max_speakers", c_int32), ("kernel_size", c_int32), ("depth", c_int32),
                ("stride_list", c_int32 * 8), ("channels", c_int32), ("growth", c_int32),
                ("encoder_channels", c_int32), ("encoder_kernel_size", c_int32), ("encoder_stride", c_int32),
                ("residual_layers", c_int32), ("residual_dilation_factor", c_int32), ("num_head", c_int32),
                ("ffw_dim", c_int32), ("bottleneck_layers", c_int32), ("bottleneck_ksize", c_int32)]

    @classmethod
    def from_config(cls, cfg):
        s = cls()
        s.n_mics, s.max_speakers, s.kernel_size, s.depth = cfg.n_mics, cfg.max_speakers, cfg.kernel_size, cfg.depth
        for i, v in enumerate(cfg.stride_list):
            s.stride_list[i] = v
        s.channels, s.growth = cfg.channels, int(cfg.growth)
        s.encoder_channels, s.encoder_kernel_size = cfg.encoder_channels, cfg.encoder_kernel_size
        s.encoder_stride, s.residual_layers = cfg.encoder_stride, cfg.residual_layers
        s.residual_dilation_factor, s.num_head = cfg.residual_dilation_factor, cfg.num_head
        s.ffw_dim, s.bottleneck_layers, s.bottleneck_ksize = cfg.ffw_dim, cfg.bottleneck_layers, cfg.bottleneck_ksize
        return s


class ConvGemmArgs(Structure):
    _fields_ = [("A", c_void_p), ("A2", c_void_p), ("Wt", c_void_p), ("bias", c_void_p),
                ("resid", c_void_p), ("mul", c_void_p), ("ln_gamma", c_void_p), ("ln_beta", c_void_p),
                ("out", c_void_p), ("stats", c_void_p),
                ("B", c_int32), ("M_out", c_int32), ("N", c_int32), ("Cin", c_int32), ("taps", c_int32),
                ("stride", c_int32), ("dil", c_int32), ("pad", c_int32), ("a_row_stride", c_int32),
                ("a_batch_stride", c_int64), ("a_len", c_int64), ("chan_mod", c_int32), ("relu", c_int32),
                ("ln_eps", c_float), ("precision", c_int32), ("w_shift", c_int32), ("Wt_hi", c_void_p),
                ("Wt_lo", c_void_p), ("Wf_hi", c_void_p), ("Wf_lo", c_void_p), ("stats_stride", c_int32),
                ("glu_raw", c_void_p), ("glu_mr", c_void_p), ("glu_gamma", c_void_p), ("glu_beta", c_void_p),
                ("glu_out", c_void_p)]


class MaskPathArgs(Structure):
    _fields_ = [("enc", ConvGemmArgs), ("ref", c_void_p), ("ref_batch_stride", c_int64), ("ref_len", c_int64),
                ("ref_hop", c_int32), ("byp_k", c_int32), ("byp_taps", c_int32), ("byp_shift", c_int32),
                ("byp_hi", c_void_p), ("byp_lo", c_void_p), ("byp_bias", c_void_p), ("dec_hi", c_void_p),
                ("dec_lo", c_void_p), ("dec_shift", c_int32), ("dec_taps", c_int32), ("taps", c_void_p)]


class ResLayerDesc(Structure):
    _fields_ = [("Wf_hi", c_void_p), ("Wf_lo", c_void_p), ("bias", c_void_p), ("ln_gamma", c_void_p),
                ("ln_beta", c_void_p), ("dil", c_int32), ("w_shift", c_int32)]


class ResStackArgs(Structure):
    _fields_ = [("x", c_void_p), ("out", c_void_p), ("B", c_int32), ("T", c_int32), ("C", c_int32), ("taps", c_int32),
                ("n_layers", c_int32), ("precision", c_int32), ("ln_eps", c_float), ("layer", ResLayerDesc * 3),
                ("glu_raw", c_void_p), ("glu_mr", c_void_p), ("glu_gamma", c_void_p), ("glu_beta", c_void_p),
                ("glu_out", c_void_p)]


SIGNATURES = {
    "asw_last_error": (c_char_p, []),
    "asw_abi_version": (c_int, []),
    "asw_profile_enable": (c_int, [c_int]),
    "asw_profile_report": (c_int, [c_char_p, c_size_t]),
    "asw_spot_create": (c_int, [POINTER(SpotConfigC), POINTER(c_void_p)]),
    "asw_spot_destroy": (None, [c_void_p]),
    "asw_spot_set_param": (c_int, [c_void_p, c_char_p, c_void_p, c_size_t]),
    "asw_spot_finalize": (c_int, [c_void_p]),
    "asw_spot_set_batch": (c_int, [c_void_p, c_int]),
    "asw_spot_set_precision": (c_int, [c_void_p, c_int]),
    "asw_spot_set_lanes": (c_int, [c_void_p, c_int]),
    "asw_split_weights_f16": (c_int, [c_void_p, c_size_t, c_void_p, c_void_p, POINTER(c_int32)]),
    "asw_pack_fragments_f16": (c_int, [c_void_p, c_int, c_int, c_void_p, c_void_p, POINTER(c_int32)]),
    "asw_spot_shift_and_sep": (c_int, [c_void_p, c_void_p, c_int, c_int, c_void_p, c_int, c_int, c_int,
                                       c_void_p, c_void_p, c_int, c_void_p]),
    "asw_spot_shift_and_sep_multi": (c_int, [c_void_p, c_void_p, c_int, c_int, c_int, c_void_p, c_void_p, c_int, c_int, c_int,
                                             c_void_p, c_void_p, c_int, c_void_p]),
    "asw_spot_forward": (c_int, [c_void_p, c_void_p, c_int, c_int, c_int, POINTER(c_float), c_void_p, c_void_p]),
    "asw_spot_set_fused_mask": (c_int, [c_void_p, c_int]),
    "asw_spot_get_tap": (c_int, [c_void_p, c_char_p, c_void_p, c_size_t, POINTER(c_size_t), c_void_p]),
    "asw_sep_create": (c_int, [POINTER(SepConfigC), POINTER(c_void_p)]),
    "asw_sep_destroy": (None, [c_void_p]),
    "asw_sep_set_param": (c_int, [c_void_p, c_char_p, c_void_p, c_size_t]),
    "asw_sep_finalize": (c_int, [c_void_p]),
    "asw_sep_set_precision": (c_int, [c_void_p, c_int]),
    "asw_sep_infer": (c_int, [c_void_p, c_void_p, c_int, c_int, c_void_p, c_int, c_void_p, c_void_p]),
    "asw_sep_forward": (c_int, [c_void_p, c_void_p, c_int, c_int, c_int, c_int, c_void_p, c_void_p]),
    "asw_sep_forward_counts": (c_int, [c_void_p, c_void_p, c_int, c_int, c_int, c_int, c_void_p, c_void_p, c_void_p]),
    "asw_sep_get_config": (c_int, [c_void_p, POINTER(SepConfigC)]),
    "asw_sep_get_tap": (c_int, [c_void_p, c_char_p, c_void_p, c_size_t, POINTER(c_size_t), c_void_p]),
    "asw_joint_shift_stats": (c_int, [c_void_p, c_int, c_int, c_void_p, c_int, c_void_p, c_void_p, c_void_p, c_void_p]),
    "asw_joint_shift_stats_scratch_doubles": (c_int, []),
    "asw_add_layernorm2": (c_int, [c_void_p, c_void_p, c_float, c_void_p, c_void_p, c_int, c_int, c_float, c_int,
                                   c_void_p, c_void_p, c_void_p]),
    "asw_glu_rows": (c_int, [c_void_p, c_long, c_int, c_void_p, c_void_p]),
    "asw_dwconv_ln_swish": (c_int, [c_void_p, c_void_p, c_void_p, c_void_p, c_void_p, c_int, c_int, c_int, c_int,
                                    c_float, c_void_p, c_void_p]),
    "asw_relpos_attention": (c_int, [c_void_p, c_void_p, c_void_p, c_void_p, c_int, c_int, c_int, c_int, c_float,
                                     c_void_p, c_void_p]),
    "asw_inter_attention": (c_int, [c_void_p, c_int, c_int, c_int, c_int, c_int, c_void_p, c_void_p]),
    "asw_shift_stats": (c_int, [c_void_p, c_int, c_int, c_void_p, c_int, c_int, c_void_p, c_void_p, c_void_p]),
    "asw_shift_norm_preproc": (c_int, [c_void_p, c_int, c_int, c_int, c_void_p, c_int, c_int, c_void_p, c_void_p,
                                       c_void_p, c_void_p, c_int, c_void_p, c_void_p, c_long, c_void_p]),
    "asw_shift_stats_multi": (c_int, [c_void_p, c_int, c_int, c_void_p, c_void_p, c_int, c_int, c_void_p, c_void_p, c_void_p]),
    "asw_shift_norm_preproc_multi": (c_int, [c_void_p, c_int, c_int, c_int, c_void_p, c_void_p, c_int, c_int, c_void_p,
                                             c_void_p, c_void_p, c_void_p, c_int, c_void_p, c_void_p, c_long, c_void_p]),
    "asw_pad_preproc": (c_int, [c_void_p, c_int, c_int, c_int, c_int, c_void_p, c_void_p, c_int, c_void_p,
                                c_void_p, c_long, c_void_p]),
    "asw_convgemm_f32": (c_int, [POINTER(ConvGemmArgs), c_void_p]),
    "asw_mask_path_f16x3": (c_int, [POINTER(MaskPathArgs), c_void_p]),
    "asw_resstack64_f16x3": (c_int, [POINTER(ResStackArgs), c_void_p]),
    "asw_convgemm_stats_tiles": (c_int, [c_int, c_int]),
    "asw_f16x3_overflow_count": (c_int, [c_int, POINTER(c_int32)]),
    "asw_gn_glu": (c_int, [c_void_p, c_void_p, c_int, c_void_p, c_void_p, c_int, c_int, c_int, c_float, c_void_p,
                           c_void_p]),
    "asw_gn_finalize": (c_int, [c_void_p, c_int, c_int, c_int, c_int, c_float, c_void_p, c_void_p]),
    "asw_attention": (c_int, [c_void_p, c_int, c_int, c_int, c_int, c_void_p, c_void_p]),
    "asw_attention_prec": (c_int, [c_void_p, c_int, c_int, c_int, c_int, c_int, c_void_p, c_void_p]),
    "asw_overlap_add_unnorm": (c_int, [c_void_p, c_int, c_int, c_int, c_int, c_int, c_int, c_int, c_int, c_float,
                                       c_void_p, c_void_p, c_void_p, c_void_p]),
    "asw_overlap_add_parts": (c_int, [c_void_p, c_int, c_int, c_int, c_int, c_int, c_int, c_int, c_int, c_int, c_float,
                                      c_void_p, c_void_p, c_void_p, c_void_p]),
    "asw_energies": (c_int, [c_void_p, c_int, c_int, c_int, c_void_p, c_void_p, c_void_p]),
    "asw_pair_sisdr": (c_int, [c_void_p, c_int, c_int, c_void_p, c_void_p]),
    "asw_center_rows": (c_int, [c_void_p, c_int, c_int, c_void_p]),
    "asw_segment_sisdr": (c_int, [c_void_p, c_int, c_int, c_void_p, c_void_p, c_int, c_void_p, c_void_p]),
    "asw_add_layernorm": (c_int, [c_void_p, c_void_p, c_void_p, c_void_p, c_int, c_int, c_float, c_void_p, c_void_p]),
    "asw_search_area": (c_int, [c_void_p, c_int, c_void_p, c_int, c_void_p, c_void_p, c_void_p, c_double, c_double,
                                POINTER(c_int), POINTER(c_void_p), POINTER(c_void_p), POINTER(c_void_p),
                                POINTER(c_void_p)]),
    "asw_free": (None, [c_void_p]),
    "asw_cube_select": (c_int, [c_void_p, c_int, c_int, c_int, c_int, c_int, c_int, c_int, c_int, c_void_p, c_void_p,
                                c_void_p, c_int64, POINTER(c_int64)]),
    "asw_cube_select_planes": (c_int, [c_void_p, c_int, c_int, c_int, c_int, c_int, c_int, c_int, c_int, c_void_p, c_void_p,
                                c_void_p, c_int64, POINTER(c_int64)]),
    "asw_srp_frames": (c_int, [c_int, c_int, c_int]),
    "asw_srp_cross_spectra": (c_int, [c_void_p, c_int, c_int, c_int, c_int, c_int, c_int, c_int, c_int, c_int,
                                      c_float, c_void_p, c_void_p, c_void_p, c_int, c_void_p, c_void_p, c_void_p]),
    "asw_srp_map": (c_int, [c_void_p, c_int, c_int, c_int, c_void_p, c_int, c_int, c_void_p, c_void_p, c_void_p,
                            c_void_p, c_void_p, c_void_p]),
    "asw_pruner_covariance": (c_int, [c_void_p, c_int, c_int, c_int, c_int, c_int, c_int, c_int, c_int, c_int,
                                      c_void_p, c_void_p, c_void_p]),
    "asw_hermitian_eigh": (c_int, [c_void_p, c_int, c_int, c_void_p, c_void_p, c_void_p]),
    "asw_music_map": (c_int, [c_void_p, c_int, c_int, c_int, c_void_p, c_int, c_void_p, c_void_p, c_void_p, c_void_p,
                              c_void_p]),
    "asw_tops_map": (c_int, [c_void_p, c_void_p, c_int, c_int, c_int, c_int, c_void_p, c_int, c_double, c_void_p,
                             c_void_p, c_void_p, c_void_p]),
    "asw_geom_lookup_planes": (c_int, [c_void_p, c_int, c_void_p, c_int, c_void_p, c_int, c_void_p, c_int, c_double, c_double,
                                       c_void_p, c_void_p]),
    "asw_geom_voxel_map": (c_int, [c_void_p, c_int, c_void_p, c_int, c_void_p, c_int, c_void_p, c_int, c_void_p, c_void_p,
                                   c_double, c_double, c_double, c_void_p, c_void_p, c_void_p, c_void_p]),
    "asw_geom_label": (c_int, [c_void_p, c_void_p, c_int, c_int, c_int, c_int, c_void_p, c_void_p, c_void_p, POINTER(c_int),
                               c_void_p]),
    "asw_geom_workspace_bytes": (c_int64, [c_int]),
    "asw_geom_compact": (c_int, [c_void_p, c_void_p, c_void_p, c_int, c_void_p, c_int, c_void_p, c_int, c_void_p, c_int,
                                 c_void_p, c_double, c_void_p, c_int64, c_void_p, c_void_p, c_void_p, c_void_p, c_void_p,
                                 c_void_p, c_void_p, c_void_p, c_void_p, POINTER(c_int), c_void_p]),
}

_lib = None


def lib():
    global _lib
    if _lib is None:
        if not os.path.exists(LIB_PATH):
            raise RuntimeError(
                f"{LIB_PATH} is missing: run `python -c 'import __graft_entry__ as g; g.build()'` "
                "(hipcc --offload-arch=gfx950).  There is no CPU fallback for the hot path.")
        import torch
        L = ctypes.CDLL(LIB_PATH)
        for name, (res, args) in SIGNATURES.items():
            fn = getattr(L, name)
            fn.restype = res
            fn.argtypes = args
        _lib = L
    return _lib


_ops = None


def torch_ops():
    global _ops
    if _ops is None:
        lib()
        if not os.path.exists(OPS_PATH):
            raise RuntimeError(f"{OPS_PATH} is missing: run `python -c 'import __graft_entry__ as g; g.build()'`.  "
                               "The hot path is exposed only through these custom ops; there is no fallback.")
        import torch
        torch.ops.load_library(OPS_PATH)
        _ops = torch.ops.asw
    return _ops


def check(status: int):
    if status != 0:
        msg = lib().asw_last_error()
        raise RuntimeError(f"libasw_hip: status {status}: {msg.decode() if msg else ''}")


def ptr(t):
    return None if t is None else c_void_p(t.data_ptr())


def current_stream():
    import torch
    return c_void_p(torch.cuda.current_stream().cuda_stream)


def to_device(a, device):
    import torch
    src = torch.from_numpy(a)
    host = torch.empty(src.shape, dtype=src.dtype, pin_memory=True)
    host.copy_(src)
    return host.to(device, non_blocking=True)


def to_host(t):
    import torch
    if not t.is_cuda:
        return t.numpy()
    host = torch.empty(t.shape, dtype=t.dtype, pin_memory=True)
    host.copy_(t)
    return host.numpy()
```

acousticswarms-speech_amd/ops.py:

```python
from ctypes import byref

import torch

from .native import ConvGemmArgs, MaskPathArgs, ResStackArgs, check, current_stream, lib, ptr


def _f32(t):
    assert t.is_cuda and t.dtype == torch.float32 and t.is_contiguous(), "need contiguous float32 CUDA tensor"
    return t


def pack_conv_weight(w: torch.Tensor) -> torch.Tensor:
    N, Cin, K = w.shape
    return w.permute(0, 2, 1).reshape(N, K * Cin).contiguous()


def convgemm(A, Wt, M_out, N, Cin, taps=1, stride=1, dil=1, pad=0, bias=None, relu=False, resid=None, mul=None,
             ln=None, stats_chan_mod=0, A2=None, B=None, a_row_stride=None, a_batch_stride=None, a_len=None,
             out=None, ln_eps=1e-5, precision="f32", use_fragments=True, glu=None, glu_out=None):
    _f32(A); _f32(Wt)
    if B is None:
        B = A.shape[0]
    a_row_stride = Cin if a_row_stride is None else a_row_stride
    if a_batch_stride is None:
        a_batch_stride = A[0].numel()
    if a_len is None:
        a_len = a_batch_stride
    if out is None:
        out = torch.empty((B, M_out, N), dtype=torch.float32, device=A.device)
    stats = None
    if stats_chan_mod:
        tiles = lib().asw_convgemm_stats_tiles(M_out, N)
        stats = torch.zeros((B, tiles, 4), dtype=torch.float32, device=A.device)
    a = ConvGemmArgs()
    a.A, a.A2, a.Wt = A.data_ptr(), (A2.data_ptr() if A2 is not None else None), Wt.data_ptr()
    a.bias = bias.data_ptr() if bias is not None else None
    a.resid = resid.data_ptr() if resid is not None else None
    a.mul = mul.data_ptr() if mul is not None else None
    a.ln_gamma = ln[0].data_ptr() if ln is not None else None
    a.ln_beta = ln[1].data_ptr() if ln is not None else None
    a.out = out.data_ptr()
    a.stats = stats.data_ptr() if stats is not None else None
    a.B, a.M_out, a.N, a.Cin, a.taps, a.stride, a.dil, a.pad = B, M_out, N, Cin, taps, stride, dil, pad
    a.a_row_stride, a.a_batch_stride, a.a_len = a_row_stride, a_batch_stride, a_len
    a.chan_mod, a.relu, a.ln_eps = stats_chan_mod, int(relu), ln_eps
    if glu is not None:
        a.glu_raw, a.glu_mr, a.glu_gamma, a.glu_beta = (_f32(t).data_ptr() for t in glu)
        if glu_out is not None:
            a.glu_out = _f32(glu_out).data_ptr()
    keep = None
    if precision in ("f16x3", "f16"):
        hi, lo, shift = split_weights_f16(Wt)
        keep = (hi, lo)
        a.precision, a.w_shift, a.Wt_hi, a.Wt_lo = (1 if precision == "f16x3" else 2), shift, hi.data_ptr(), lo.data_ptr()
        if use_fragments and N % 32 == 0 and (taps * Cin) % 16 == 0:
            fh, fl, sh2 = pack_fragments_f16(Wt, N, taps * Cin)
            assert sh2 == shift
            keep = keep + (fh, fl)
            a.Wf_hi, a.Wf_lo = fh.data_ptr(), fl.data_ptr()
    check(lib().asw_convgemm_f32(byref(a), current_stream()))
    torch.cuda.current_stream().synchronize() if keep is not None else None
    return out, stats


def resstack(x, layers, taps=7, precision="f16x3", eps=1e-5, glu=None, out=None, glu_out=None):
    src = x if glu is None else glu[0]
    B, T = src.shape[0], src.shape[1]
    if out is None:
        out = torch.empty((B, T, 64), dtype=torch.float32, device=src.device)
    a = ResStackArgs()
    a.x = _f32(x).data_ptr() if x is not None else None
    a.out = out.data_ptr()
    a.B, a.T, a.C, a.taps, a.n_layers = B, T, 64, taps, len(layers)
    a.precision, a.ln_eps = (1 if precision == "f16x3" else 2), eps
    keep = []
    for i, (Wt, bias, gamma, beta, dil) in enumerate(layers):
        fh, fl, sh = pack_fragments_f16(_f32(Wt), 64, taps * 64)
        keep.append((fh, fl))
        d = a.layer[i]
        d.Wf_hi, d.Wf_lo, d.w_shift, d.dil = fh.data_ptr(), fl.data_ptr(), sh, dil
        d.bias, d.ln_gamma, d.ln_beta = _f32(bias).data_ptr(), _f32(gamma).data_ptr(), _f32(beta).data_ptr()
    if glu is not None:
        a.glu_raw, a.glu_mr, a.glu_gamma, a.glu_beta = (_f32(t).data_ptr() for t in glu)
        if glu_out is not None:
            a.glu_out = _f32(glu_out).data_ptr()
    check(lib().asw_resstack64_f16x3(byref(a), current_stream()))
    torch.cuda.current_stream().synchronize()
    return out


def pack_fragments_f16(Wt, N, K):
    import ctypes
    import numpy as np
    w = np.ascontiguousarray(Wt.detach().cpu().numpy(), dtype=np.float32).reshape(N, K)
    hi = np.empty(w.size, dtype=np.uint16)
    lo = np.empty(w.size, dtype=np.uint16)
    sh = ctypes.c_int32()
    check(lib().asw_pack_fragments_f16(ctypes.c_void_p(w.ctypes.data), N, K, ctypes.c_void_p(hi.ctypes.data),
                                       ctypes.c_void_p(lo.ctypes.data), byref(sh)))
    dev = Wt.device
    return (torch.from_numpy(hi.view(np.int16)).to(dev), torch.from_numpy(lo.view(np.int16)).to(dev), sh.value)


def split_weights_f16(Wt):
    import ctypes
    import numpy as np
    w = np.ascontiguousarray(Wt.detach().cpu().numpy(), dtype=np.float32)
    hi = np.empty(w.size, dtype=np.uint16)
    lo = np.empty(w.size, dtype=np.uint16)
    sh = ctypes.c_int32()
    check(lib().asw_split_weights_f16(ctypes.c_void_p(w.ctypes.data), w.size, ctypes.c_void_p(hi.ctypes.data),
                                      ctypes.c_void_p(lo.ctypes.data), byref(sh)))
    dev = Wt.device
    return (torch.from_numpy(hi.view(np.int16)).to(dev), torch.from_numpy(lo.view(np.int16)).to(dev), sh.value)


def gn_glu(raw, stats, gamma, beta, eps=1e-5):
    B, T, C2 = raw.shape
    C = C2 // 2
    out = torch.empty((B, T, C), dtype=torch.float32, device=raw.device)
    check(lib().asw_gn_glu(ptr(_f32(raw)), ptr(_f32(stats)), stats.shape[1], ptr(_f32(gamma)), ptr(_f32(beta)),
                           B, T, C, eps, ptr(out), current_stream()))
    return out


def gn_finalize(stats, T, C, eps=1e-5):
    B = stats.shape[0]
    mr = torch.empty((B, 4), dtype=torch.float32, device=stats.device)
    check(lib().asw_gn_finalize(ptr(_f32(stats)), stats.shape[1], B, T, C, eps, ptr(mr), current_stream()))
    return mr


def add_layernorm(x, resid, gamma, beta, eps=1e-5):
    rows, N = x.shape
    out = torch.empty_like(x)
    check(lib().asw_add_layernorm(ptr(_f32(x)), ptr(_f32(resid)), ptr(_f32(gamma)), ptr(_f32(beta)), rows, N, eps,
                                  ptr(out), current_stream()))
    return out


def attention(qkv, nhead, precision="f32"):
    B, L, d3 = qkv.shape
    d = d3 // 3
    ctx = torch.empty((B, L, d), dtype=torch.float32, device=qkv.device)
    check(lib().asw_attention_prec(ptr(_f32(qkv)), B, L, d, nhead, {"f32": 0, "f16x3": 1, "f16": 2}[precision], ptr(ctx),
                                   current_stream()))
    return ctx


def shift_stats(mix, offsets, circular=True):
    M, T = mix.shape
    N = offsets.shape[0]
    mean = torch.empty((N,), dtype=torch.float32, device=mix.device)
    std = torch.empty((N,), dtype=torch.float32, device=mix.device)
    check(lib().asw_shift_stats(ptr(_f32(mix)), M, T, ptr(offsets), N, int(circular), ptr(mean), ptr(std),
                                current_stream()))
    return mean, std


def shift_norm_preproc(mix, offsets, mean, std, w, b, T_pad, circular=True):
    M, T = mix.shape
    N = offsets.shape[0]
    C = w.shape[0]
    x0 = torch.empty((N, T_pad, C), dtype=torch.float32, device=mix.device)
    refn = torch.zeros((N, T_pad), dtype=torch.float32, device=mix.device)
    check(lib().asw_shift_norm_preproc(ptr(_f32(mix)), M, T, T_pad, ptr(offsets), N, int(circular), ptr(mean),
                                       ptr(std), ptr(_f32(w)), ptr(_f32(b)), C, ptr(x0), ptr(refn), T_pad,
                                       current_stream()))
    return x0, refn


def overlap_add_unnorm(D, taps, hop, t, trim_left, trim_right, bias, mean=None, std=None):
    B, F, ldd = D.shape
    out = torch.empty((B, t), dtype=torch.float32, device=D.device)
    check(lib().asw_overlap_add_unnorm(ptr(_f32(D)), B, F, ldd, taps, hop, t, trim_left, trim_right, float(bias),
                                       ptr(mean), ptr(std), ptr(out), current_stream()))
    return out


def overlap_add_parts(Dp, taps, hop, t, trim_left, trim_right, bias, mean=None, std=None):
    nparts, B, F, ldd = Dp.shape
    out = torch.empty((B, t), dtype=torch.float32, device=Dp.device)
    check(lib().asw_overlap_add_parts(ptr(_f32(Dp)), nparts, B, F, ldd, taps, hop, t, trim_left, trim_right,
                                      float(bias), ptr(mean), ptr(std), ptr(out), current_stream()))
    return out


def mask_path(x, ref, ref_hop, enc_w, enc_b, byp_w, byp_b, dec_w, frames, stride, pad):
    B, Tp, C = x.shape
    E, _, EK = enc_w.shape
    dev = x.device
    Wt = pack_conv_weight(enc_w).to(dev)
    fh, fl, sh = pack_fragments_f16(Wt, E, EK * C)
    wb = torch.zeros((E, 48), dtype=torch.float32)
    wb[:, :byp_w.shape[-1]] = byp_w[:, 0].cpu()
    bh, bl, bsh = pack_fragments_f16(wb.to(dev), E, 48)
    wd = torch.zeros((64, E), dtype=torch.float32)
    wd[:dec_w.shape[-1]] = dec_w[:, 0].t().cpu()
    dh, dl, dsh = pack_fragments_f16(wd.to(dev), 64, E)
    parts = torch.zeros((E // 256, B, frames, 64), dtype=torch.float32, device=dev)
    m = MaskPathArgs()
    a = m.enc
    a.A, a.bias = _f32(x).data_ptr(), (_f32(enc_b).data_ptr() if enc_b is not None else None)
    a.B, a.M_out, a.N, a.Cin, a.taps, a.stride, a.dil, a.pad = B, frames, E, C, EK, stride, 1, pad
    a.a_row_stride, a.a_batch_stride, a.a_len = C, Tp * C, Tp * C
    a.precision, a.w_shift, a.Wf_hi, a.Wf_lo = 1, sh, fh.data_ptr(), fl.data_ptr()
    m.ref, m.ref_batch_stride, m.ref_len, m.ref_hop = _f32(ref).data_ptr(), ref.shape[1], ref.shape[1], ref_hop
    m.byp_k, m.byp_taps, m.byp_shift = 48, byp_w.shape[-1], bsh
    m.byp_hi, m.byp_lo = bh.data_ptr(), bl.data_ptr()
    m.byp_bias = _f32(byp_b).data_ptr() if byp_b is not None else None
    m.dec_hi, m.dec_lo, m.dec_shift, m.dec_taps = dh.data_ptr(), dl.data_ptr(), dsh, dec_w.shape[-1]
    m.taps = parts.data_ptr()
    check(lib().asw_mask_path_f16x3(byref(m), current_stream()))
    torch.cuda.current_stream().synchronize()
    return parts


def energies(y, window=12000):
    B, T = y.shape
    scratch = torch.empty((B, T + 1), dtype=torch.float64, device=y.device)
    out = torch.empty((B, 2), dtype=torch.float64, device=y.device)
    check(lib().asw_energies(ptr(_f32(y)), B, T, window, ptr(scratch), ptr(out), current_stream()))
    return out


def pair_sisdr(y):
    n, T = y.shape
    out = torch.empty((n, n), dtype=torch.float64, device=y.device)
    check(lib().asw_pair_sisdr(ptr(_f32(y)), n, T, ptr(out), current_stream()))
    return out


def joint_shift_stats(mix, offsets):
    M, T = mix.shape
    S = offsets.shape[0]
    scratch = torch.empty((lib().asw_joint_shift_stats_scratch_doubles(),), dtype=torch.float64, device=mix.device)
    mean = torch.empty((S,), dtype=torch.float32, device=mix.device)
    std = torch.empty((S,), dtype=torch.float32, device=mix.device)
    check(lib().asw_joint_shift_stats(ptr(_f32(mix)), M, T, ptr(offsets), S, ptr(scratch), ptr(mean), ptr(std),
                                      current_stream()))
    return mean, std


def add_layernorm2(x, y=None, alpha=1.0, gamma=None, beta=None, eps=1e-5, act=0, want_sum=False, want_ln=True):
    rows, N = x.shape
    s = torch.empty_like(x) if want_sum else None
    o = torch.empty_like(x) if want_ln else None
    check(lib().asw_add_layernorm2(ptr(_f32(x)), ptr(y), float(alpha), ptr(gamma), ptr(beta), rows, N, eps, act, ptr(s),
                                   ptr(o), current_stream()))
    return s, o


def glu_rows(raw):
    rows, C2 = raw.shape
    out = torch.empty((rows, C2 // 2), dtype=torch.float32, device=raw.device)
    check(lib().asw_glu_rows(ptr(_f32(raw)), rows, C2 // 2, ptr(out), current_stream()))
    return out


def dwconv_ln_swish(u, w, bias, gamma, beta, eps=1e-5):
    BS, L, d = u.shape
    K = w.shape[-1]
    wT = w.reshape(d, K).t().contiguous()
    out = torch.empty_like(u)
    check(lib().asw_dwconv_ln_swish(ptr(_f32(u)), ptr(_f32(wT)), ptr(_f32(bias)), ptr(_f32(gamma)), ptr(_f32(beta)),
                                    BS, L, d, K, eps, ptr(out), current_stream()))
    return out


def relpos_attention(qkv, P, bias_u, bias_v, nhead, scale):
    BS, L, d3 = qkv.shape
    d = d3 // 3
    ctx = torch.empty((BS, L, d), dtype=torch.float32, device=qkv.device)
    check(lib().asw_relpos_attention(ptr(_f32(qkv)), ptr(_f32(P)), ptr(_f32(bias_u)), ptr(_f32(bias_v)), BS, L, d, nhead,
                                     float(scale), ptr(ctx), current_stream()))
    return ctx


def inter_attention(qkv, nhead):
    NB, S, L, d3 = qkv.shape
    d = d3 // 3
    ctx = torch.empty((NB, S, L, d), dtype=torch.float32, device=qkv.device)
    check(lib().asw_inter_attention(ptr(_f32(qkv)), NB, S, L, d, nhead, ptr(ctx), current_stream()))
    return ctx


def f16x3_overflow_count(reset=True) -> int:
    import ctypes
    c = ctypes.c_int32()
    check(lib().asw_f16x3_overflow_count(int(reset), byref(c)))
    return int(c.value) & 0xFFFFFFFF
```

include/asw_hip.h:

```cpp
#ifndef ASW_HIP_H
#define ASW_HIP_H

#include <stddef.h>
#include <stdint.h>

#ifdef __cplusplus
extern "C" {
#endif

typedef enum asw_status {
  ASW_OK = 0,
  ASW_ERR_ARG = -1,
  ASW_ERR_HIP = -2,
  ASW_ERR_NOMEM = -3,
  ASW_ERR_STATE = -4
} asw_status;

const char* asw_last_error(void);
int asw_abi_version(void);

int asw_profile_enable(int on);
int asw_profile_report(char* buf, size_t cap);

typedef struct asw_spot_config {
  int32_t n_mics;
  int32_t kernel_size;
  int32_t depth;
  int32_t stride_list[8];
  int32_t channels;
  int32_t growth;
  int32_t encoder_channels;
  int32_t encoder_kernel_size;
  int32_t encoder_stride;
  int32_t residual_layers;
  int32_t residual_dilation_factor;
  int32_t num_head;
  int32_t ffw_dim;
  int32_t num_transformer_layers;
} asw_spot_config;

typedef struct asw_spot asw_spot;

int asw_spot_create(const asw_spot_config* cfg, asw_spot** out);
void asw_spot_destroy(asw_spot* m);

int asw_spot_set_param(asw_spot* m, const char* key, const float* host_data, size_t numel);
int asw_spot_finalize(asw_spot* m);

int asw_spot_set_batch(asw_spot* m, int batch);

int asw_spot_set_lanes(asw_spot* m, int lanes);

int asw_spot_set_precision(asw_spot* m, int precision);

int asw_spot_shift_and_sep(asw_spot* m, const float* mix, int M, int T,
                           const int32_t* offsets, int N, int strict, int circular,
                           float* out_wave, double* out_energy, int energy_window,
                           void* stream);

int asw_spot_shift_and_sep_multi(asw_spot* m, const float* mix, int K, int M, int T, const int32_t* offsets,
                                 const int32_t* mix_index, int N, int strict, int circular, float* out_wave,
                                 double* out_energy, int energy_window, void* stream);

int asw_spot_forward(asw_spot* m, const float* mix_norm, int B, int M, int t,
                     const float* window_embedding_host, float* out, void* stream);

int asw_spot_set_fused_mask(asw_spot* m, int on);

int asw_spot_get_tap(asw_spot* m, const char* name, float* dst, size_t capacity, size_t* numel,
                     void* stream);

typedef struct asw_sep_config {
  int32_t n_mics;
  int32_t max_speakers;
  int32_t kernel_size;
  int32_t depth;
  int32_t stride_list[8];
  int32_t channels;
  int32_t growth;
  int32_t encoder_channels;
  int32_t encoder_kernel_size;
  int32_t encoder_stride;
  int32_t residual_layers;
  int32_t residual_dilation_factor;
  int32_t num_head;
  int32_t ffw_dim;
  int32_t bottleneck_layers;
  int32_t bottleneck_ksize;
} asw_sep_config;

typedef struct asw_sep asw_sep;

int asw_sep_create(const asw_sep_config* cfg, asw_sep** out);
void asw_sep_destroy(asw_sep* m);
int asw_sep_set_param(asw_sep* m, const char* key, const float* host_data, size_t numel);
int asw_sep_finalize(asw_sep* m);
int asw_sep_set_precision(asw_sep* m, int precision);

int asw_sep_infer(asw_sep* m, const float* mix, int M, int T, const int32_t* offsets, int S, float* out,
                  void* stream);

int asw_sep_forward(asw_sep* m, const float* mix_norm, int B, int S, int M, int t, float* out, void* stream);
int asw_sep_forward_counts(asw_sep* m, const float* mix_norm, int B, int S, int M, int t, const int32_t* counts,
                           float* out, void* stream);
int asw_sep_get_config(const asw_sep* m, asw_sep_config* out);

int asw_sep_get_tap(asw_sep* m, const char* name, float* dst, size_t capacity, size_t* numel, void* stream);

int asw_joint_shift_stats(const float* mix, int M, int T, const int32_t* offsets, int S, double* scratch,
                          float* mean, float* std, void* stream);
int asw_joint_shift_stats_scratch_doubles(void);

int asw_add_layernorm2(const float* x, const float* y, float alpha, const float* gamma, const float* beta,
                       int rows, int N, float eps, int act, float* sum_out, float* ln_out, void* stream);

int asw_glu_rows(const float* raw, long rows, int C, float* out, void* stream);

int asw_dwconv_ln_swish(const float* u, const float* wT, const float* bias, const float* gamma, const float* beta,
                        int BS, int L, int d, int K, float eps, float* out, void* stream);

int asw_relpos_attention(const float* qkv, const float* P, const float* bias_u, const float* bias_v, int BS, int L,
                         int d, int nhead, float scale, float* ctx, void* stream);

int asw_inter_attention(const float* qkv, int NB, int S, int L, int d, int nhead, float* ctx, void* stream);


int asw_shift_stats(const float* mix, int M, int T, const int32_t* offsets, int N,
                    int circular, float* mean, float* std, void* stream);

int asw_shift_norm_preproc(const float* mix, int M, int T, int T_pad, const int32_t* offsets,
                           int N, int circular, const float* mean, const float* std,
                           const float* w, const float* b, int C, float* x0, float* refn,
                           long refn_stride, void* stream);

int asw_shift_stats_multi(const float* mix, int M, int T, const int32_t* offsets, const int32_t* mix_index, int N,
                          int circular, float* mean, float* std, void* stream);
int asw_shift_norm_preproc_multi(const float* mix, int M, int T, int T_pad, const int32_t* offsets,
                                 const int32_t* mix_index, int N, int circular, const float* mean, const float* std,
                                 const float* w, const float* b, int C, float* x0, float* refn, long refn_stride,
                                 void* stream);

int asw_pad_preproc(const float* x, int B, int M, int t, int T_pad, const float* w,
                    const float* b, int C, float* x0, float* refn, long refn_stride,
                    void* stream);

typedef struct asw_convgemm_args {
  const float* A;
  const float* A2;
  const float* Wt;
  const float* bias;
  const float* resid;
  const float* mul;
  const float* ln_gamma;
  const float* ln_beta;
  float* out;
  float* stats;
  int32_t B, M_out, N, Cin, taps, stride, dil, pad;
  int32_t a_row_stride;
  int64_t a_batch_stride;
  int64_t a_len;
  int32_t chan_mod;
  int32_t relu;
  float ln_eps;
  int32_t precision;
  int32_t w_shift;
  const void* Wt_hi;
  const void* Wt_lo;
  const void* Wf_hi;
  const void* Wf_lo;
  int32_t stats_stride;
  const float* glu_raw;
  const float* glu_mr;
  const float* glu_gamma;
  const float* glu_beta;
  float* glu_out;
} asw_convgemm_args;
int asw_pack_fragments_f16(const float* Wt, int N, int K, uint16_t* hi, uint16_t* lo, int32_t* w_shift);
int asw_convgemm_f32(const asw_convgemm_args* args, void* stream);
typedef struct asw_maskpath_args {
  asw_convgemm_args enc;
  const float* ref;
  int64_t ref_batch_stride;
  int64_t ref_len;
  int32_t ref_hop;
  int32_t byp_k;
  int32_t byp_taps;
  int32_t byp_shift;
  const void* byp_hi;
  const void* byp_lo;
  const float* byp_bias;
  const void* dec_hi;
  const void* dec_lo;
  int32_t dec_shift;
  int32_t dec_taps;
  float* taps;
} asw_maskpath_args;
int asw_mask_path_f16x3(const asw_maskpath_args* args, void* stream);
typedef struct asw_reslayer_desc {
  const void* Wf_hi;
  const void* Wf_lo;
  const float* bias;
  const float* ln_gamma;
  const float* ln_beta;
  int32_t dil;
  int32_t w_shift;
} asw_reslayer_desc;
typedef struct asw_resstack_args {
  const float* x;
  float* out;
  int32_t B, T, C, taps, n_layers;
  int32_t precision;
  float ln_eps;
  asw_reslayer_desc layer[3];
  const float* glu_raw;
  const float* glu_mr;
  const float* glu_gamma;
  const float* glu_beta;
  float* glu_out;
} asw_resstack_args;
int asw_resstack64_f16x3(const asw_resstack_args* args, void* stream);
int asw_split_weights_f16(const float* w, size_t n, uint16_t* hi, uint16_t* lo, int32_t* w_shift);
int asw_f16x3_overflow_count(int reset, uint32_t* count);
int asw_convgemm_stats_tiles(int M_out, int N);

int asw_gn_glu(const float* raw, const float* stats, int n_partials, const float* gamma,
               const float* beta, int B, int T, int C, float eps, float* out, void* stream);
int asw_gn_finalize(const float* stats, int n_partials, int B, int T, int C, float eps, float* mr, void* stream);

int asw_attention(const float* qkv, int B, int L, int d, int nhead, float* ctx, void* stream);
int asw_attention_prec(const float* qkv, int B, int L, int d, int nhead, int precision, float* ctx, void* stream);

int asw_overlap_add_unnorm(const float* D, int B, int F, int ldd, int taps, int hop,
                           int t, int trim_left, int trim_right, float bias, const float* mean,
                           const float* std, float* out, void* stream);
int asw_overlap_add_parts(const float* D, int nparts, int B, int F, int ldd, int taps, int hop,
                          int t, int trim_left, int trim_right, float bias, const float* mean,
                          const float* std, float* out, void* stream);

int asw_energies(const float* y, int B, int T, int window, double* scratch, double* out,
                 void* stream);

int asw_add_layernorm(const float* x, const float* resid, const float* gamma, const float* beta,
                      int rows, int N, float eps, float* out, void* stream);

int asw_center_rows(float* y, int B, int T, void* stream);

int asw_pair_sisdr(const float* y, int n, int T, double* out, void* stream);

int asw_segment_sisdr(const float* y, int n, int T, const int32_t* segments, const int32_t* seg_count,
                      int kmax, double* out, void* stream);

int asw_search_area(const double* points, int n_pts, const double* mic, int M, double* offset,
                    double* width, const double* ub, double sound_speed, double fs, int* n_children,
                    double** child_offset, double** child_width, int** child_count, int** child_index);
void asw_free(void* p);

int asw_cube_select(const double* offsets, int ny, int nx, int nz, int P, int y0, int y1, int x0, int x1,
                    const double* lo, const double* hi, int32_t* out_idx, int64_t cap, int64_t* count);
int asw_cube_select_planes(const double* planes, int ny, int nx, int nz, int P, int y0, int y1, int x0, int x1,
                    const double* lo, const double* hi, int32_t* out_idx, int64_t cap, int64_t* count);

int asw_srp_frames(int window, int nfft, int hop);
int asw_srp_cross_spectra(const float* mix, int M, int T, int window, int step, int n_windows,
                          int nfft, int hop, int nbins, int nb_pad, float tol,
                          const float* twiddle, const int32_t* pair_i, const int32_t* pair_j,
                          int P, float* xf_scratch, float* cc, void* stream);
int asw_srp_map(const float* cc, int n_windows, int nbins, int P, const double* tau, int G, int M,
                const double* omega, const int32_t* pair_i, const int32_t* pair_j,
                float* part_scratch, float* out, void* stream);

int asw_pruner_covariance(const float* mix, int M, int T, int window, int step, int n_windows,
                          int nfft, int hop, int bin0, int nbins, double* cov, double* magsum,
                          void* stream);
int asw_hermitian_eigh(const double* a, int n, int M, double* evals, double* evecs, void* stream);
int asw_music_map(const double* evecs, int n_windows, int nbins, int M, const double* tau, int G,
                  const double* omega, double* p_scratch, double* max_scratch, float* out,
                  void* stream);
int asw_tops_map(const double* evecs, const double* magsum, int n_windows, int nbins, int bin0,
                 int M, const double* delta, int G, double coef, double* q_scratch,
                 int32_t* max_bin, float* out, void* stream);

int asw_geom_lookup_planes(const double* ys, int ny, const double* xs, int nx, const double* zs, int nz,
                           const double* mics, int M, double C, double FS, double* planes, void* stream);
int asw_geom_voxel_map(const double* xs, int Lx, const double* ys, int Ly, const double* zs, int Lz,
                       const double* mics, int M, const double* border, const double* centre, double C,
                       double FS, double resolution, int32_t* q, uint8_t* valid, double* dis_matrix,
                       void* stream);
int asw_geom_label(const int32_t* q, const uint8_t* valid, int Lx, int Ly, int Lz, int P,
                   uint32_t* adj_scratch, int32_t* flag_scratch, int32_t* labels, int* sweeps, void* stream);
int64_t asw_geom_workspace_bytes(int n_voxels);
int asw_geom_compact(const int32_t* labels, const int32_t* q, const double* xs, int Lx, const double* ys, int Ly,
                     const double* zs, int Lz, const double* mics, int M, const double* centre, double C,
                     void* workspace, int64_t workspace_bytes, int32_t* power_index, int32_t* valid_flat,
                     int32_t* valid_cid, int32_t* members, int32_t* bounds, int32_t* offsets, double* centres,
                     double* tau, double* delta, int* counts, void* stream);

#ifdef __cplusplus
}
#endif
#endif
```

Baseline: 2383 candidates/s.

## Fuse shift/normalise preprocessing into the first encoder residual stack load

The shift, quantise, normalise and 1x1 preprocessing conv is now computed inside the first fused resstack kernel's tile-loading stage, reading the raw mixture directly. The separate preproc kernel and its full B x T x 64 activation write and read-back are skipped, and refn is written as a side output. This removes one kernel launch and a large round trip through memory at the cost of recomputing the preprocessing for halo rows and extra registers in the load stage. It is enabled by default when M<=8 and channels are 64.

Result: no change. 2397 candidates/s, median of 6 (+0.6%).

```diff
diff --git a/acousticswarms-speech_amd/csrc/asw_common.h b/acousticswarms-speech_amd/csrc/asw_common.h
--- a/acousticswarms-speech_amd/csrc/asw_common.h
+++ b/acousticswarms-speech_amd/csrc/asw_common.h
@@ -50,6 +50,20 @@
   const float e = __builtin_amdgcn_exp2f(__fmul_rn(gv, -1.4426950408889634f));
   return __fmul_rn(av, __builtin_amdgcn_rcpf(__fadd_rn(1.0f, e)));
 }
+
+__device__ __forceinline__ float quant16(float x) { return rintf(x * 32768.0f) * (1.0f / 32768.0f); }
+__device__ __forceinline__ int shifted_index(int t, int off, int T, int circular) {
+  const int i = t + off;
+  if (circular) return i >= T ? i - T : i;
+  return (i >= 0 && i < T) ? i : -1;
+}
+__device__ __forceinline__ float quant_norm(float x, float mu, float sg) { return (quant16(x) - mu) / sg; }
+__device__ __forceinline__ void preproc_fma(float4& o, float w0, float w1, float w2, float w3, float x) {
+  o.x = fmaf(w0, x, o.x);
+  o.y = fmaf(w1, x, o.y);
+  o.z = fmaf(w2, x, o.z);
+  o.w = fmaf(w3, x, o.w);
+}
 #endif
 
 }
diff --git a/acousticswarms-speech_amd/csrc/model_common.h b/acousticswarms-speech_amd/csrc/model_common.h
--- a/acousticswarms-speech_amd/csrc/model_common.h
+++ b/acousticswarms-speech_amd/csrc/model_common.h
@@ -150,8 +150,22 @@
   return true;
 }
 
+inline bool stage_fusion(char part) {
+  static const char* env = getenv("ASW_STAGE_FUSION");
+  if (!env || !*env) return true;
+  if (env[0] == '0') return false;
+  if (env[0] == 'a' || env[0] == 'A' || env[0] == 'b' || env[0] == 'B') return (env[0] | 0x20) == part;
+  return true;
+}
+
+struct PreSrc {
+  const float* mix; const int32_t* offsets; const int32_t* mix_index; const float *mean, *stdv, *w, *b;
+  float* refn; long refn_stride; int M, T, circular;
+};
+
 inline int run_res(const std::vector<ResLayer>& res, int prec, int B, int T, int ch, int K, float* x, float* p, float* q,
-            float** final_out, hipStream_t s, const GluSrc* glu = nullptr) {
+            float** final_out, hipStream_t s, const GluSrc* glu = nullptr, const PreSrc* pre = nullptr) {
+  if (pre && !resstack_ok(res, prec, ch, K)) return asw::set_error(ASW_ERR_STATE, "run_res: the preproc source needs the fused stack");
   const float* in = glu ? glu->raw : x;
   float* outb = p;
   if (resstack_ok(res, prec, ch, K)) {
@@ -166,8 +180,9 @@
         halo += pad;
         ++n;
       }
-      asw_resstack_args a = {};
-      a.x = (glu && j == 0) ? nullptr : in;
+      asw_resstack_src_args sa = {};
+      asw_resstack_args& a = sa.stack;
+      a.x = ((glu || pre) && j == 0) ? nullptr : in;
       a.out = outb;
       a.B = B; a.T = T; a.C = ch; a.taps = K; a.n_layers = (int)n; a.precision = prec; a.ln_eps = 1e-5f;
       for (size_t i = 0; i < n; ++i) {
@@ -178,7 +193,16 @@
       if (glu && j == 0) {
         a.glu_raw = glu->raw; a.glu_mr = glu->mr; a.glu_gamma = glu->gamma; a.glu_beta = glu->beta; a.glu_out = glu->side_out;
       }
-      int rc = asw_resstack64_f16x3(&a, s);
+      int rc;
+      if (pre && j == 0) {
+        sa.pre_mix = pre->mix; sa.pre_offsets = pre->offsets; sa.pre_mix_index = pre->mix_index;
+        sa.pre_mean = pre->mean; sa.pre_std = pre->stdv; sa.pre_w = pre->w; sa.pre_b = pre->b;
+        sa.pre_refn = pre->refn; sa.pre_refn_stride = pre->refn_stride;
+        sa.pre_M = pre->M; sa.pre_T = pre->T; sa.pre_circular = pre->circular;
+        rc = asw_resstack64_src_f16x3(&sa, s);
+      } else {
+        rc = asw_resstack64_f16x3(&a, s);
+      }
       if (rc) return rc;
       in = outb;
       outb = (outb == p) ? q : p;
@@ -278,6 +302,7 @@
   float *mean, *stdv, *refn;
   std::vector<float*> X, Pb, Qb, raw_dn, raw_up, st_dn, st_up, mr_dn, mr_up;
   float *Y, *D, *ywave;
+  const PreSrc* pre = nullptr;
 };
 
 struct Trunk {
@@ -504,17 +529,21 @@
     pl.ywave = a.take<float>((size_t)pl.B * pl.T);
   }
 
+  bool preproc_on_load_ok(int M) const {
+    return stage_fusion('a') && M <= 8 && tc.channels == 64 && resstack_ok(enc[0].res, precision, tc.channels, tc.kernel_size);
+  }
+
   int encode(TrunkPlan& pl, const GatedConvs& g, hipStream_t s) {
     const int B = pl.B, K = tc.kernel_size;
     taps.clear();
-    taps["preproc"] = {pl.X[0], (size_t)B * pl.Tl[0] * tc.channels};
+    if (!pl.pre) taps["preproc"] = {pl.X[0], (size_t)B * pl.Tl[0] * tc.channels};
     int rc;
     GluSrc src = {};
     bool glu = false;
     for (int i = 0; i < tc.depth; ++i) {
       float* r = nullptr;
       if ((rc = run_res(enc[i].res, precision, B, pl.Tl[i], enc_cin[i], K, pl.X[i], pl.Pb[i], pl.Qb[i], &r, s,
-                        glu ? &src : nullptr)))
+                        glu ? &src : nullptr, i == 0 ? pl.pre : nullptr)))
         return rc;
       asw_convgemm_args a = {};
       a.A = r; g.down_wt[i].bind(a, precision); a.bias = enc[i].bias.p; a.out = pl.raw_dn[i]; a.stats = pl.st_dn[i];
diff --git a/acousticswarms-speech_amd/csrc/prep_kernels.hip b/acousticswarms-speech_amd/csrc/prep_kernels.hip
--- a/acousticswarms-speech_amd/csrc/prep_kernels.hip
+++ b/acousticswarms-speech_amd/csrc/prep_kernels.hip
@@ -4,9 +4,7 @@
 
 constexpr int MAX_MICS = 32;
 
-__device__ __forceinline__ float quant16(float x) {
-  return rintf(x * 32768.0f) * (1.0f / 32768.0f);
-}
+using asw::quant16;
 
 __device__ __forceinline__ double block_sum(double v, double* red) {
 #pragma unroll
@@ -97,10 +95,8 @@
     if (tp >= pad && tp < T_pad) {
       const int t = tp - pad;
       if (SHIFTED) {
-        int i = t + off[m];
-        if (circular) { if (i >= T) i -= T; x = src[(long)m * T + i]; }
-        else x = (i >= 0 && i < T) ? src[(long)m * T + i] : 0.f;
-        x = (quant16(x) - mu) / sg;
+        const int i = asw::shifted_index(t, off[m], T, circular);
+        x = asw::quant_norm(i >= 0 ? src[(long)m * T + i] : 0.f, mu, sg);
       } else {
         x = src[((long)n * M + m) * T + t];
       }
@@ -117,11 +113,7 @@
     float4 o = *reinterpret_cast<const float4*>(bias + c);
     if (tp >= pad) {
       for (int m = 0; m < M; ++m) {
-        const float x = vs[r * M + m];
-        o.x = fmaf(ws[(c + 0) * M + m], x, o.x);
-        o.y = fmaf(ws[(c + 1) * M + m], x, o.y);
-        o.z = fmaf(ws[(c + 2) * M + m], x, o.z);
-        o.w = fmaf(ws[(c + 3) * M + m], x, o.w);
+        asw::preproc_fma(o, ws[(c + 0) * M + m], ws[(c + 1) * M + m], ws[(c + 2) * M + m], ws[(c + 3) * M + m], vs[r * M + m]);
       }
     }
     *reinterpret_cast<float4*>(x0 + ((long)n * T_pad + tp) * C + c) = o;
diff --git a/acousticswarms-speech_amd/csrc/resstack.hip b/acousticswarms-speech_amd/csrc/resstack.hip
--- a/acousticswarms-speech_amd/csrc/resstack.hip
+++ b/acousticswarms-speech_amd/csrc/resstack.hip
@@ -38,6 +38,16 @@
   const float* glu_gamma;
   const float* glu_beta;
   float* glu_out;
+  const float* pre_mix;
+  const int32_t* pre_off;
+  const int32_t* pre_mi;
+  const float* pre_mean;
+  const float* pre_std;
+  const float* pre_w;
+  const float* pre_b;
+  float* pre_refn;
+  long pre_refn_stride;
+  int pre_M, pre_Ts, pre_circ;
   int B, T, taps, ntile, BM, img_rows;
   float eps;
   LayerDev L[MAXL];
@@ -95,11 +105,14 @@
   }
 }
 
-template <int NL, int NW, int TM, int PH, bool POLY, bool GLU, int NTERM, int QD>
+constexpr int PRE_MAXM = 8;
+
+template <int NL, int NW, int TM, int PH, bool POLY, bool GLU, bool PRE, int NTERM, int QD>
 __global__ __launch_bounds__(64 * NW) __attribute__((amdgpu_waves_per_eu(TM >= 4 ? 1 : 2)))
 void resstack64_kernel(const KArgs p) {
   static_assert(!POLY || NL == 1, "polyphase row sets: single layers only");
   static_assert(QD == 2 || QD == 4, "weight prefetch depth in k-steps");
+  static_assert(!PRE || (!POLY && !GLU), "preproc on load: contiguous tiles of a plain input");
   constexpr int NTHR = 64 * NW, SROWS = NTHR / 16;
   constexpr int R0 = 32 * NW * TM;
   constexpr int BMJ = R0 / PH;
@@ -129,7 +142,73 @@
     const float* src = w == 0 ? p.L[li].bias : w == 1 ? p.L[li].gamma : p.L[li].beta;
     reinterpret_cast<float4*>(tab)[i] = *reinterpret_cast<const float4*>(src + c4 * 4);
   }
-  {
+  if constexpr (PRE) {
+    const int srow = tid >> 4, sc4 = tid & 15;
+    const int M = p.pre_M, Ts = p.pre_Ts, padl = T - Ts;
+    const __amdgpu_buffer_rsrc_t rM = act_rsrc(p.pre_mix + (p.pre_mi ? (long)p.pre_mi[b] * M * Ts : 0), (long)M * Ts);
+    int off = 0;
+    if (sc4 > 0 && sc4 < M) {
+      off = p.pre_off[(long)b * (M - 1) + sc4 - 1];
+      if (p.pre_circ) { off %= Ts; if (off < 0) off += Ts; }
+    }
+    const float mu = p.pre_mean[b], sg = p.pre_std[b];
+    const float4 bias4 = *reinterpret_cast<const float4*>(p.pre_b + sc4 * 4);
+    const __amdgpu_buffer_rsrc_t rW = act_rsrc(p.pre_w, (long)C * M);
+    float w[4][PRE_MAXM];
+#pragma unroll
+    for (int j = 0; j < 4; ++j)
+#pragma unroll
+      for (int m = 0; m < PRE_MAXM; ++m)
+        w[j][m] = __builtin_bit_cast(float, __builtin_amdgcn_raw_buffer_load_b32(
+            rW, m < M ? ((sc4 * 4 + j) * M + m) * 4 : (int)0x80000000, 0, 0));
+    constexpr int SU = 18;
+    for (int r0 = 0; r0 < R_img; r0 += SROWS * SU) {
+      float xs[SU];
+#pragma unroll
+      for (int u = 0; u < SU; ++u) {
+        const int row = r0 + u * SROWS + srow;
+        const int g = m0 - p.L[0].halo - pad0 + row;
+        const bool ok = row < R_img && g >= padl && g < T && sc4 < M;
+        const int i = asw::shifted_index(g - padl, off, Ts, p.pre_circ);
+        const int v = __builtin_amdgcn_raw_buffer_load_b32(rM, (ok && i >= 0) ? (sc4 * Ts + i) * 4 : (int)0x80000000, 0, 0);
+        xs[u] = __builtin_bit_cast(float, v);
+      }
+#pragma unroll
+      for (int u = 0; u < SU; ++u) {
+        const int row = r0 + u * SROWS + srow;
+        const int g = m0 - p.L[0].halo - pad0 + row;
+        const bool ok = row < R_img && g >= padl && g < T && sc4 < M;
+        xs[u] = ok ? asw::quant_norm(xs[u], mu, sg) : 0.f;
+      }
+#pragma unroll
+      for (int u = 0; u < SU; ++u) {
+        const int row = r0 + u * SROWS + srow;
+        const int g = m0 - p.L[0].halo - pad0 + row;
+        float4 o = bias4;
+#pragma unroll
+        for (int m = 0; m < PRE_MAXM; ++m) {
+          const float xm = __shfl(xs[u], m, 16);
+          asw::preproc_fma(o, w[0][m], w[1][m], w[2][m], w[3][m], xm);
+        }
+        if (g < padl) o = bias4;
+        if (g < 0 || g >= T) o = make_float4(0.f, 0.f, 0.f, 0.f);
+        if (row < R_img) {
+          half4 hi, lo;
+          split4t<NTERM>(o, hi, lo);
+          *reinterpret_cast<half4*>(img + row * RS + sc4 * 8) = hi;
+          *reinterpret_cast<half4*>(img + row * RS + 128 + sc4 * 8) = lo;
+        }
+      }
+      if (p.pre_refn && sc4 == 0) {
+#pragma unroll
+        for (int u = 0; u < SU; ++u) {
+          const int row = r0 + u * SROWS + srow;
+          const int g = m0 - p.L[0].halo - pad0 + row;
+          if (row < R_img && g >= m0 && g < m0 + p.BM && g < T) p.pre_refn[(long)b * p.pre_refn_stride + g] = xs[u];
+        }
+      }
+    }
+  } else {
     const __amdgpu_buffer_rsrc_t rX = GLU ? act_rsrc(p.glu_raw + (long)b * T * 2 * C, (long)T * 2 * C)
                                           : act_rsrc(p.x + (long)b * T * C, (long)T * C);
     const int srow = tid >> 4, sc4 = tid & 15;
@@ -376,30 +455,30 @@
 #endif
 }
 
-template <int NL, int NW, int TM, int PH, bool POLY, bool GLU, int QD>
+template <int NL, int NW, int TM, int PH, bool POLY, bool GLU, int QD, bool PRE = false>
 int launch_stack(const KArgs& k, int precision, size_t smem, double flops, const char* tag, hipStream_t s) {
   const bool x1 = precision == 2;
-  auto kern = x1 ? resstack64_kernel<NL, NW, TM, PH, POLY, GLU, 1, QD> : resstack64_kernel<NL, NW, TM, PH, POLY, GLU, 3, QD>;
+  auto kern = x1 ? resstack64_kernel<NL, NW, TM, PH, POLY, GLU, PRE, 1, QD> : resstack64_kernel<NL, NW, TM, PH, POLY, GLU, PRE, 3, QD>;
   static asw::SmemAttr attr[2];
   if (int rc = attr[x1].ensure(reinterpret_cast<const void*>(kern), 160 * 1024)) return rc;
   const int total = k.B * k.ntile;
   dim3 grid(((total + 7) / 8) * 8);
   char nm[128];
   int nl = snprintf(nm, sizeof nm, "resstack64<%s,%dx%d%s%s>", tag, NW, TM, POLY ? (PH == 1 ? ",poly1" : PH == 2 ? ",poly2" : ",poly4") : "",
-                    GLU ? ",glu" : "");
+                    GLU ? ",glu" : PRE ? ",pre" : "");
   if (asw::prof_detail()) snprintf(nm + nl, sizeof nm - nl, "[B%d M%d d%d]", k.B, k.T, k.L[0].dil);
-  asw::ProfScope prof(s, nm, flops, (double)k.B * k.T * C * 4 * (GLU ? 3 : 2));
+  asw::ProfScope prof(s, nm, flops, (double)k.B * k.T * C * 4 * (GLU ? 3 : PRE ? 1 : 2));
   hipLaunchKernelGGL(kern, grid, dim3(64 * NW), smem, s, k);
   ASW_LAUNCH_CHECK();
   return ASW_OK;
 }
 
 template <int NW, int TM>
-int dispatch(const asw_resstack_args& a, KArgs& k, bool glu, double flops, hipStream_t s) {
+int dispatch(const asw_resstack_args& a, KArgs& k, bool glu, bool pre, double flops, hipStream_t s) {
   constexpr int R0 = 32 * NW * TM;
   const int dil0 = k.L[0].dil;
   const int rpp = a.T / dil0;
-  if (a.n_layers == 1 && dil0 >= 7 && rpp >= 48 && !glu) {
+  if (a.n_layers == 1 && dil0 >= 7 && rpp >= 48 && !glu && !pre) {
     const int PH = rpp >= R0 - 32 ? 1 : rpp >= R0 / 2 - 32 ? 2 : 4;
     const int BMJ = R0 / PH;
     k.BM = R0;
@@ -427,6 +506,16 @@
   const size_t smem = (size_t)rows * RS + (size_t)a.n_layers * 3 * 64 * sizeof(float);
   ASW_CHECK_ARG(smem <= 160 * 1024, "resstack: image of %d rows exceeds LDS (dilation %d x %d taps too wide for a contiguous tile)",
                 rows, dil0, a.taps);
+  if (pre) {
+    if constexpr (NW == 4 && TM == 2) {
+      switch (a.n_layers) {
+        case 1: return launch_stack<1, NW, TM, 1, false, false, 4, true>(k, a.precision, smem, flops, "1", s);
+        case 2: return launch_stack<2, NW, TM, 1, false, false, 4, true>(k, a.precision, smem, flops, "2", s);
+        default: return launch_stack<3, NW, TM, 1, false, false, 4, true>(k, a.precision, smem, flops, "3", s);
+      }
+    }
+    return asw::set_error(ASW_ERR_ARG, "resstack: the preproc source runs on the 4x2 tile only");
+  }
   switch (a.n_layers) {
     case 1: return glu ? launch_stack<1, NW, TM, 1, false, true, 4>(k, a.precision, smem, flops, "1", s)
                        : launch_stack<1, NW, TM, 1, false, false, 4>(k, a.precision, smem, flops, "1", s);
@@ -450,21 +539,36 @@
 }
 #endif
 
-extern "C" int asw_resstack64_f16x3(const asw_resstack_args* args, void* stream) {
-  ASW_CHECK_ARG(args != nullptr, "resstack: null args");
-  const asw_resstack_args& a = *args;
+namespace {
+int run_stack(const asw_resstack_args& a, const asw_resstack_src_args* src, void* stream) {
   hipStream_t s = asw::as_stream(stream);
+  const bool pre = src != nullptr;
   ASW_CHECK_ARG(a.C == C, "resstack: C=%d (64 only)", a.C);
   ASW_CHECK_ARG(a.n_layers >= 1 && a.n_layers <= MAXL, "resstack: 1..%d layers", MAXL);
   ASW_CHECK_ARG(a.taps >= 3 && a.taps <= 15 && a.taps % 2 == 1, "resstack: taps=%d (odd, 3..15)", a.taps);
   ASW_CHECK_ARG(a.precision == 1 || a.precision == 2, "resstack: precision 1 (f16x3) or 2 (single-pass f16)");
   ASW_CHECK_ARG(a.B > 0 && a.B <= (1 << 20) && a.T > 0 && (int64_t)a.T * 2 * C < ((int64_t)1 << 29), "resstack: bad B / T");
-  ASW_CHECK_ARG(a.out && (a.x || a.glu_raw), "resstack: null tensor");
+  ASW_CHECK_ARG(a.out && (a.x || a.glu_raw || pre), "resstack: null tensor");
   const bool glu = a.glu_raw != nullptr;
+  if (pre) {
+    ASW_CHECK_ARG(!a.x && !glu, "resstack: the preproc source replaces x / glu_raw");
+    ASW_CHECK_ARG(src->pre_mix && src->pre_offsets && src->pre_mean && src->pre_std && src->pre_w && src->pre_b,
+                  "resstack: preproc source incomplete");
+    ASW_CHECK_ARG(src->pre_M >= 1 && src->pre_M <= PRE_MAXM && src->pre_T >= 1 && src->pre_T <= a.T,
+                  "resstack: preproc source M=%d (1..%d), T=%d of %d padded rows", src->pre_M, PRE_MAXM, src->pre_T, a.T);
+    ASW_CHECK_ARG((int64_t)src->pre_M * src->pre_T < ((int64_t)1 << 28), "resstack: mixture too long for one buffer descriptor");
+    ASW_CHECK_ARG(!src->pre_refn || src->pre_refn_stride >= a.T, "resstack: pre_refn_stride < T");
+  }
   if (glu) ASW_CHECK_ARG(a.glu_mr && a.glu_gamma && a.glu_beta, "resstack: GroupNorm + GLU on load needs the statistics / affine arrays");
   KArgs k = {};
   k.x = a.x; k.out = a.out; k.glu_raw = a.glu_raw; k.glu_mr = a.glu_mr; k.glu_gamma = a.glu_gamma; k.glu_beta = a.glu_beta;
   k.glu_out = glu ? a.glu_out : nullptr;
+  if (pre) {
+    k.pre_mix = src->pre_mix; k.pre_off = src->pre_offsets; k.pre_mi = src->pre_mix_index;
+    k.pre_mean = src->pre_mean; k.pre_std = src->pre_std; k.pre_w = src->pre_w; k.pre_b = src->pre_b;
+    k.pre_refn = src->pre_refn; k.pre_refn_stride = (long)src->pre_refn_stride;
+    k.pre_M = src->pre_M; k.pre_Ts = src->pre_T; k.pre_circ = src->pre_circular;
+  }
   k.B = a.B; k.T = a.T; k.taps = a.taps; k.eps = a.ln_eps;
   int halo = 0;
   for (int i = a.n_layers - 1; i >= 0; --i) {
@@ -479,11 +583,23 @@
   }
   const double flops = 2.0 * a.B * (double)a.T * C * C * a.taps * a.n_layers;
   static const int tile_env = getenv("ASW_RESSTACK_TILE") ? atoi(getenv("ASW_RESSTACK_TILE")) : 0;
-  const int variant = tile_env == 24 || tile_env == 44 || tile_env == 82 ? tile_env : 42;
+  const int variant = (tile_env == 24 || tile_env == 44 || tile_env == 82) && !pre ? tile_env : 42;
   switch (variant) {
-    case 24: return dispatch<2, 4>(a, k, glu, flops, s);
-    case 44: return dispatch<4, 4>(a, k, glu, flops, s);
-    case 82: return dispatch<8, 2>(a, k, glu, flops, s);
-    default: return dispatch<4, 2>(a, k, glu, flops, s);
-  }
-}
+    case 24: return dispatch<2, 4>(a, k, glu, pre, flops, s);
+    case 44: return dispatch<4, 4>(a, k, glu, pre, flops, s);
+    case 82: return dispatch<8, 2>(a, k, glu, pre, flops, s);
+    default: return dispatch<4, 2>(a, k, glu, pre, flops, s);
+  }
+}
+}
+
+extern "C" int asw_resstack64_f16x3(const asw_resstack_args* args, void* stream) {
+  ASW_CHECK_ARG(args != nullptr, "resstack: null args");
+  return run_stack(*args, nullptr, stream);
+}
+
+extern "C" int asw_resstack64_src_f16x3(const asw_resstack_src_args* args, void* stream) {
+  ASW_CHECK_ARG(args != nullptr, "resstack: null args");
+  ASW_CHECK_ARG(args->pre_mix != nullptr, "resstack: no source given (pre_mix)");
+  return run_stack(args->stack, args, stream);
+}
diff --git a/acousticswarms-speech_amd/csrc/spot_model.hip b/acousticswarms-speech_amd/csrc/spot_model.hip
--- a/acousticswarms-speech_amd/csrc/spot_model.hip
+++ b/acousticswarms-speech_amd/csrc/spot_model.hip
@@ -277,8 +277,10 @@
       ASW_HIP(hipMemsetAsync(p.refn, 0, (size_t)B * p.RL * sizeof(float), q));
       int r;
       if ((r = asw_shift_stats_multi(mix, M, T, off, mi, B, circular, p.mean, p.stdv, q))) return r;
-      if ((r = asw_shift_norm_preproc_multi(mix, M, T, p.Tp, off, mi, B, circular, p.mean, p.stdv, m->pre_w.p, m->pre_b.p, C,
-                                            p.X[0], p.refn + pad_l, p.RL, q)))
+      const PreSrc pre = {mix, off, mi, p.mean, p.stdv, m->pre_w.p, m->pre_b.p, p.refn + pad_l, p.RL, M, T, circular};
+      p.pre = m->preproc_on_load_ok(M) ? &pre : nullptr;
+      if (!p.pre && (r = asw_shift_norm_preproc_multi(mix, M, T, p.Tp, off, mi, B, circular, p.mean, p.stdv, m->pre_w.p,
+                                                      m->pre_b.p, C, p.X[0], p.refn + pad_l, p.RL, q)))
         return r;
       float* y = out_wave ? out_wave + (size_t)i0 * T : p.ywave;
       if ((r = run_network(m, p, gs, p.mean, p.stdv, y, q))) return r;
diff --git a/acousticswarms-speech_amd/native.py b/acousticswarms-speech_amd/native.py
--- a/acousticswarms-speech_amd/native.py
+++ b/acousticswarms-speech_amd/native.py
@@ -136,6 +136,13 @@
                 ("n_layers", c_int32), ("precision", c_int32), ("ln_eps", c_float), ("layer", ResLayerDesc * 3),
                 ("glu_raw", c_void_p), ("glu_mr", c_void_p), ("glu_gamma", c_void_p), ("glu_beta", c_void_p),
                 ("glu_out", c_void_p)]
+
+
+class ResStackSrcArgs(Structure):
+    _fields_ = [("stack", ResStackArgs), ("pre_mix", c_void_p), ("pre_offsets", c_void_p), ("pre_mix_index", c_void_p),
+                ("pre_mean", c_void_p), ("pre_std", c_void_p), ("pre_w", c_void_p), ("pre_b", c_void_p),
+                ("pre_refn", c_void_p), ("pre_refn_stride", c_int64), ("pre_M", c_int32), ("pre_T", c_int32),
+                ("pre_circular", c_int32)]
 
 
 SIGNATURES = {
@@ -190,6 +197,7 @@
     "asw_convgemm_f32": (c_int, [POINTER(ConvGemmArgs), c_void_p]),
     "asw_mask_path_f16x3": (c_int, [POINTER(MaskPathArgs), c_void_p]),
     "asw_resstack64_f16x3": (c_int, [POINTER(ResStackArgs), c_void_p]),
+    "asw_resstack64_src_f16x3": (c_int, [POINTER(ResStackSrcArgs), c_void_p]),
     "asw_convgemm_stats_tiles": (c_int, [c_int, c_int]),
     "asw_f16x3_overflow_count": (c_int, [c_int, POINTER(c_int32)]),
     "asw_gn_glu": (c_int, [c_void_p, c_void_p, c_int, c_void_p, c_void_p, c_int, c_int, c_int, c_float, c_void_p,
diff --git a/acousticswarms-speech_amd/ops.py b/acousticswarms-speech_amd/ops.py
--- a/acousticswarms-speech_amd/ops.py
+++ b/acousticswarms-speech_amd/ops.py
@@ -2,7 +2,7 @@
 
 import torch
 
-from .native import ConvGemmArgs, MaskPathArgs, ResStackArgs, check, current_stream, lib, ptr
+from .native import ConvGemmArgs, MaskPathArgs, ResStackArgs, ResStackSrcArgs, check, current_stream, lib, ptr
 
 
 def _f32(t):
@@ -63,12 +63,19 @@
     return out, stats
 
 
-def resstack(x, layers, taps=7, precision="f16x3", eps=1e-5, glu=None, out=None, glu_out=None):
-    src = x if glu is None else glu[0]
-    B, T = src.shape[0], src.shape[1]
+def resstack(x, layers, taps=7, precision="f16x3", eps=1e-5, glu=None, out=None, glu_out=None, preproc=None):
+    if preproc is not None:
+        assert x is None and glu is None
+        src = preproc["mix"]
+        B, T = preproc["offsets"].shape[0], int(preproc["T_pad"])
+        sa = ResStackSrcArgs()
+        a = sa.stack
+    else:
+        src = x if glu is None else glu[0]
+        B, T = src.shape[0], src.shape[1]
+        a = ResStackArgs()
     if out is None:
         out = torch.empty((B, T, 64), dtype=torch.float32, device=src.device)
-    a = ResStackArgs()
     a.x = _f32(x).data_ptr() if x is not None else None
     a.out = out.data_ptr()
     a.B, a.T, a.C, a.taps, a.n_layers = B, T, 64, taps, len(layers)
@@ -84,7 +91,24 @@
         a.glu_raw, a.glu_mr, a.glu_gamma, a.glu_beta = (_f32(t).data_ptr() for t in glu)
         if glu_out is not None:
             a.glu_out = _f32(glu_out).data_ptr()
-    check(lib().asw_resstack64_f16x3(byref(a), current_stream()))
+    if preproc is not None:
+        q = preproc
+        offs = q["offsets"]
+        assert offs.is_cuda and offs.dtype == torch.int32 and offs.is_contiguous()
+        sa.pre_mix, sa.pre_offsets = _f32(q["mix"]).data_ptr(), offs.data_ptr()
+        mi = q.get("mix_index")
+        if mi is not None:
+            assert mi.is_cuda and mi.dtype == torch.int32 and mi.is_contiguous()
+            sa.pre_mix_index = mi.data_ptr()
+        sa.pre_mean, sa.pre_std = _f32(q["mean"]).data_ptr(), _f32(q["std"]).data_ptr()
+        sa.pre_w, sa.pre_b = _f32(q["w"]).data_ptr(), _f32(q["b"]).data_ptr()
+        refn = q.get("refn")
+        if refn is not None:
+            sa.pre_refn, sa.pre_refn_stride = _f32(refn).data_ptr(), refn.shape[1]
+        sa.pre_M, sa.pre_T, sa.pre_circular = q["mix"].shape[-2], q["mix"].shape[-1], int(q.get("circular", True))
+        check(lib().asw_resstack64_src_f16x3(byref(sa), current_stream()))
+    else:
+        check(lib().asw_resstack64_f16x3(byref(a), current_stream()))
     torch.cuda.current_stream().synchronize()
     return out
 
diff --git a/include/asw_hip.h b/include/asw_hip.h
--- a/include/asw_hip.h
+++ b/include/asw_hip.h
@@ -219,6 +219,20 @@
   float* glu_out;
 } asw_resstack_args;
 int asw_resstack64_f16x3(const asw_resstack_args* args, void* stream);
+typedef struct asw_resstack_src_args {
+  asw_resstack_args stack;
+  const float* pre_mix;
+  const int32_t* pre_offsets;
+  const int32_t* pre_mix_index;
+  const float* pre_mean;
+  const float* pre_std;
+  const float* pre_w;
+  const float* pre_b;
+  float* pre_refn;
+  int64_t pre_refn_stride;
+  int32_t pre_M, pre_T, pre_circular;
+} asw_resstack_src_args;
+int asw_resstack64_src_f16x3(const asw_resstack_src_args* args, void* stream);
 int asw_split_weights_f16(const float* w, size_t n, uint16_t* hi, uint16_t* lo, int32_t* w_shift);
 int asw_f16x3_overflow_count(int reset, uint32_t* count);
 int asw_convgemm_stats_tiles(int M_out, int N);
```
